# bacpop/ska.rust

Measured on AMD Instinct MI355X. Metric: genomes/sec ska build+align, 1 000x5 Mbp k=31; bit-exact vs CPU, higher is better.
Workload: dtype u64

## Files before the change

ska.rust_amd/csrc/skx_append.hip:

```cpp
#include "skx_device.h"
#include <cstdlib>
#include <type_traits>

namespace skx {

typedef uint32_t u32x4 __attribute__((ext_vector_type(4)));
typedef const u32x4 __attribute__((address_space(1))) *g4_t;

#ifdef SKX_AP_PROF
__device__ unsigned long long g_ap_prof[16];
#define AP_PROF_START unsigned long long tprof = __builtin_readcyclecounter(), tacc[12] = {0, 0, 0, 0, 0, 0, 0, 0, 0, 0, 0, 0}
#define AP_PROF(i) do { const unsigned long long t_ = __builtin_readcyclecounter(); tacc[(i)] += t_ - tprof; tprof = t_; } while (0)
#define AP_PROF_FLUSH() do { for (int i_ = 0; i_ < 12; i_++) if (tacc[i_] && (i_ >= 6 || (threadIdx.x & 63) == 0)) atomicAdd(&g_ap_prof[i_], tacc[i_]); } while (0)
extern "C" void skx_debug_phase_prof(unsigned long long *out, int reset)
{
    unsigned long long h[16];
    (void)hipDeviceSynchronize();
    (void)hipMemcpyFromSymbol(h, HIP_SYMBOL(g_ap_prof), sizeof(h));
    for (int i = 0; i < 16; i++) out[i] = h[i];
    if (reset) { for (auto &x : h) x = 0; (void)hipMemcpyToSymbol(HIP_SYMBOL(g_ap_prof), h, sizeof(h)); }
}
#else
#define AP_PROF_START do { } while (0)
#define AP_PROF(i) do { } while (0)
#define AP_PROF_FLUSH() do { } while (0)
#endif
#ifdef SKX_AP_PROF
#define AP_COUNT(i, v) do { tacc[(i)] += (v); } while (0)
#else
#define AP_COUNT(i, v) do { } while (0)
#endif

#ifndef AP_PRIO_L
#define AP_PRIO_L 1
#endif
#ifndef AP_PRIO_I
#define AP_PRIO_I 0
#endif
constexpr int AP_PRIO_STREAM = 3, AP_PRIO_LOOKUP = AP_PRIO_L, AP_PRIO_INSERT = AP_PRIO_I;
constexpr int AP_THREADS = 1024, AP_WAVES = 16;
constexpr uint32_t AP_PAD = 64;
constexpr uint32_t AP_Q = 256, AP_SQ = 64;
#ifndef AP_CH_N
#define AP_CH_N 8
#endif
#ifndef AP_RESYNC
#define AP_RESYNC 16
#endif
constexpr int AP_CH = AP_CH_N;
constexpr int AP_RANK_BITS = 14;
constexpr uint32_t AP_RANK_MASK = (1u << AP_RANK_BITS) - 1;

__device__ static inline uint32_t ap_wave_excl(uint32_t v, uint32_t *total)
{
    uint32_t inc = v;
#pragma unroll
    for (int d = 1; d < 64; d <<= 1) { const uint32_t t = __shfl_up(inc, d, 64); if ((int)(threadIdx.x & 63) >= d) inc += t; }
    *total = __shfl(inc, 63, 64);
    return inc - v;
}
__device__ static inline uint32_t ap_block_excl(uint32_t v, uint32_t *s_tmp , uint32_t *total)
{
    const int lane = threadIdx.x & 63, wv = threadIdx.x >> 6, nw = (blockDim.x + 63) >> 6;
    uint32_t wt;
    const uint32_t ex = ap_wave_excl(v, &wt);
    if (lane == 63) s_tmp[wv] = wt;
    __syncthreads();
    if (threadIdx.x == 0) { uint32_t run = 0; for (int i = 0; i < nw; i++) { const uint32_t t = s_tmp[i]; s_tmp[i] = run; run += t; } s_tmp[16] = run; }
    __syncthreads();
    const uint32_t r = s_tmp[wv] + ex;
    *total = s_tmp[16];
    __syncthreads();
    return r;
}
__device__ static inline uint32_t ap_mbcnt(unsigned long long b)
{
    return __builtin_amdgcn_mbcnt_hi((uint32_t)(b >> 32), __builtin_amdgcn_mbcnt_lo((uint32_t)b, 0u));
}

typedef volatile uint32_t __attribute__((address_space(3))) *lds_vol_t;
__device__ static inline lds_vol_t lds_vol(void *p) { return (lds_vol_t)(__attribute__((address_space(3))) void *)p; }
constexpr int CTL_NROWS = 0, CTL_FAIL = 1, CTL_TMP = 8, CTL_WORDS = 32;

static inline size_t append_lds_bytes(uint32_t nslots, uint32_t cap, bool count_only)
{
    size_t b = (size_t)(nslots + AP_PAD) * 8 + (size_t)(nslots + AP_PAD) + (size_t)AP_WAVES * (AP_Q + AP_SQ) * 8 + CTL_WORDS * 4;
    if (!count_only) b += (size_t)AP_WAVES * (cap / 8) * 4;
    return b;
}

template <bool COUNT_ONLY, bool HI>
__global__ __launch_bounds__(AP_THREADS) void append_kernel(AppendArgs a)
{
    extern __shared__ __attribute__((aligned(16))) unsigned char s_raw[];
    const uint32_t total_slots = a.nslots + AP_PAD;
    const uint32_t cap = a.cap, rbw = cap / 8;
    unsigned char *s_fp = s_raw;
    unsigned long long *s_tab = reinterpret_cast<unsigned long long *>(s_raw + total_slots);
    unsigned long long *s_q = s_tab + total_slots;
    uint32_t *s_ctl = reinterpret_cast<uint32_t *>(s_q + (size_t)AP_WAVES * (AP_Q + AP_SQ));
    uint32_t *s_rb = s_ctl + CTL_WORDS;
    const int tid = threadIdx.x, lane = tid & 63;
    const int wv = __builtin_amdgcn_readfirstlane(tid >> 6);
    const int S = a.n_samples;
    const int shA = a.logQ - a.logB;
    const uint32_t A = 1u << shA;
    const uint32_t G = gridDim.x;
    const bool xmap = a.logB >= 3 && G % (8u * A) == 0u;
    const int rem = a.bits - a.logQ;
    const int psh = rem + 4;
    const int lowb = HI ? rem - 32 : 0;
    const uint32_t fmask = HI ? (A - 1u) << (psh - 32) : 0u;
    uint32_t region = 0, part = 0, pshift = 0;
    uint64_t j = 0;
    uint8_t *piece0 = nullptr;
    unsigned long long *q = s_q + (size_t)wv * (AP_Q + AP_SQ), *sq = q + AP_Q;
    uint32_t *rb = s_rb + (size_t)wv * rbw;
    for (uint32_t rnd = 0; rnd < a.rounds; rnd++) {
    if (xmap) {
        const uint32_t xcd = blockIdx.x & 7u, ls = blockIdx.x >> 3, gpr = (G >> 3) >> shA;
        region = ((rnd * gpr + (ls >> shA)) << 3) + xcd; part = ls & (A - 1u);
    } else { const uint32_t blk = rnd * G + blockIdx.x; region = blk >> shA; part = blk & (A - 1u); }
    j = ((uint64_t)region << shA) + part;
    pshift = HI ? part << (psh - 32) : 0u;
    piece0 = a.pieces + j * (uint64_t)S * (cap / 2);

    for (uint32_t i = tid; i < total_slots; i += AP_THREADS) s_tab[i] = 0ull;
    for (uint32_t i = tid; i < total_slots / 4u; i += AP_THREADS) reinterpret_cast<uint32_t *>(s_fp)[i] = 0u;
    if (!COUNT_ONLY) for (uint32_t i = tid; i < AP_WAVES * rbw; i += AP_THREADS) s_rb[i] = 0u;
    if (tid < CTL_WORDS) s_ctl[tid] = 0u;
    if (tid == 0 && (uint32_t)(uintptr_t)(__attribute__((address_space(3))) unsigned char *)s_fp != 0u) atomicOr(a.overflow, 4);
    if (xmap && A > 1u && a.bar && tid == 0) {
        atomicAdd(&a.bar[region], 1);
        for (int it = 0; it < (1 << 18) && __hip_atomic_load(&a.bar[region], __ATOMIC_RELAXED, __HIP_MEMORY_SCOPE_AGENT) < (int)A; it++) __builtin_amdgcn_s_sleep(8);
    }
    __syncthreads();

    typedef const uint64_t __attribute__((address_space(4))) *cq_t;
    typedef const uint32_t __attribute__((address_space(4))) *c1_t;
    cq_t c_off = (cq_t)(uintptr_t)a.off;
    c1_t c_raw = (c1_t)(uintptr_t)a.raw;
    const uint64_t rstride = 1ull << a.logB;
    const uint32_t qbase = (uint32_t)(uintptr_t)(__attribute__((address_space(3))) unsigned long long *)q, qfull = qbase + 128u * 8u;
    uint32_t qw = qbase, nsq = 0;
    AP_PROF_START;
    __builtin_amdgcn_s_setprio(AP_PRIO_STREAM);

    auto key_hi = [&](uint32_t wlo, uint32_t whi) -> uint32_t {
        if (HI) return __builtin_amdgcn_alignbit(whi, wlo, (uint32_t)(rem - 28));
        return rem == 0 ? 0u : (uint32_t)(((wlo >> 4) | (whi << 28)) << (32 - rem));
    };
    const uint32_t hshift = (uint32_t)__builtin_clz(a.nslots) + 1u;
    auto home = [&](uint32_t kh) -> uint32_t { return kh >> hshift; };
    auto key_lo = [&](uint32_t wlo) -> uint32_t { return HI ? __builtin_amdgcn_ubfe(wlo, 4u, (uint32_t)lowb) << AP_RANK_BITS : 0u; };
    auto key_fp = [&](uint32_t kh, uint32_t kl) -> uint32_t {
        const uint32_t v = HI ? kh & 0xFFu : ((kh ^ (kl >> AP_RANK_BITS)) * 0x9E3779B1u) >> 24;
        return v | 1u;
    };
    auto record = [&](uint32_t rank1, uint32_t m4) {
        const uint32_t rank = rank1 - 1u;
        atomicOr(&rb[rank >> 3], m4 << ((rank & 7u) * 4u));
    };
    auto slow_batch = [&]() {
        __builtin_amdgcn_s_setprio(AP_PRIO_INSERT);
        const uint32_t take = nsq < 64u ? nsq : 64u;
        nsq -= take;
        if (lane == 0) { AP_COUNT(8, 1); AP_COUNT(9, take); }
        if ((uint32_t)lane < take) {
            const unsigned long long w = sq[nsq + lane];
            const uint32_t wlo = (uint32_t)w, whi = (uint32_t)(w >> 32);
            const uint32_t kh = key_hi(wlo, whi), kl = key_lo(wlo);
            const unsigned long long keyE = ((unsigned long long)kh << 32) | kl;
            uint32_t rank1 = 0;
            for (uint32_t t = home(kh); t + 3u < total_slots;) {
                AP_COUNT(10, 1); if (ap_mbcnt(__ballot(true)) == 0u) AP_COUNT(11, 1);
                const unsigned long long e0 = s_tab[t], e1 = s_tab[t + 1], e2 = s_tab[t + 2], e3 = s_tab[t + 3];
                const bool m0 = (e0 ^ keyE) - 1ull < AP_RANK_MASK, m1 = (e1 ^ keyE) - 1ull < AP_RANK_MASK, m2 = (e2 ^ keyE) - 1ull < AP_RANK_MASK, m3 = (e3 ^ keyE) - 1ull < AP_RANK_MASK;
                bool won = false;
                uint32_t at = 0;
                if (!(m0 | m1 | m2 | m3)) {
                    at = e0 == 0ull ? 0u : e1 == 0ull ? 1u : e2 == 0ull ? 2u : e3 == 0ull ? 3u : 4u;
                    if (at < 4u) won = atomicCAS(&s_tab[t + at], 0ull, keyE | AP_RANK_MASK) == 0ull;
                }
                if (won) {
                    const uint32_t mine = atomicAdd(&s_ctl[CTL_NROWS], 1u) + 1u;
                    if (mine > (COUNT_ONLY ? AP_RANK_MASK - 1u : cap)) s_ctl[CTL_FAIL] = 1u;
                    lds_vol(&s_tab[t + at])[0] = kl | (mine < AP_RANK_MASK ? mine : AP_RANK_MASK - 1u);
                    s_fp[t + at] = (unsigned char)key_fp(kh, kl);
                    rank1 = mine;
                }
                __builtin_amdgcn_wave_barrier();
                if (m0 | m1 | m2 | m3) {
                    const uint32_t mt = t + (m0 ? 0u : m1 ? 1u : m2 ? 2u : 3u);
                    uint32_t r = (uint32_t)(m0 ? e0 : m1 ? e1 : m2 ? e2 : e3) & AP_RANK_MASK;
                    for (int it = 0; it < (1 << 16) && r == AP_RANK_MASK; it++) r = lds_vol(&s_tab[mt])[0] & AP_RANK_MASK;
                    if (r == AP_RANK_MASK) { s_ctl[CTL_FAIL] = 1u; r = 0; }
                    rank1 = r;
                    break;
                }
                if (won) break;
                if (at == 4u) t += 4u;
            }
            if (rank1 > cap && !COUNT_ONLY) rank1 = 0;
            if (rank1 == 0) s_ctl[CTL_FAIL] = 1u;
            else if (!COUNT_ONLY) record(rank1, wlo & 15u);
        }
        __builtin_amdgcn_s_setprio(AP_PRIO_STREAM);
    };
    auto batch = [&](auto full_tag) {
        constexpr bool FULL = decltype(full_tag)::value;
        __builtin_amdgcn_s_setprio(AP_PRIO_LOOKUP);
        uint32_t nq = (qw - qbase) >> 3;
        const uint32_t take = FULL ? 128u : nq < 128u ? nq : 128u;
        nq -= take;
        qw -= take * 8u;
        if (lane == 0) { AP_COUNT(6, 1); AP_COUNT(7, take); }
        const bool va = FULL || (uint32_t)lane < take, vb = FULL || (uint32_t)lane + 64u < take;
        unsigned long long wa = 0, wb = 0;
        if (va) wa = q[nq + lane];
        if (vb) wb = q[nq + 64u + lane];
        const uint32_t alo = (uint32_t)wa, ahi = (uint32_t)(wa >> 32), blo = (uint32_t)wb, bhi = (uint32_t)(wb >> 32);
        const uint32_t kha = key_hi(alo, ahi), kla = key_lo(alo), khb = key_hi(blo, bhi), klb = key_lo(blo);
        const uint32_t hsa = home(kha), hsb = home(khb);
        auto where8 = [&](uint32_t hs, uint32_t fp) -> uint32_t {
            typedef const uint32_t __attribute__((address_space(3))) *lds_c32_t;
            const lds_c32_t f = (lds_c32_t)(uintptr_t)(hs & ~3u);
            const uint32_t fp4 = __builtin_amdgcn_perm(fp, fp, 0u);
            const uint32_t x0 = f[0] ^ fp4, x1 = f[1] ^ fp4;
            const uint32_t hs8 = hs << 3;
            const uint32_t z0 = (x0 - 0x01010101u) & ~x0 & (0x80808080u << (hs8 & 31u)), z1 = (x1 - 0x01010101u) & ~x1 & 0x80808080u;
            uint32_t p0, p1;
            asm("v_ffbl_b32 %0, %1" : "=v"(p0) : "v"(z0));
            asm("v_ffbl_b32 %0, %1" : "=v"(p1) : "v"(z1));
            p1 |= 32u;
            const uint32_t p = (p0 < p1 ? p0 : p1) & ~7u;
            return (hs8 & ~31u) + (p < 64u ? p : 64u);
        };
        const uint32_t oa = where8(hsa, key_fp(kha, kla)), ob = where8(hsb, key_fp(khb, klb));
        const unsigned long long ea = *reinterpret_cast<const unsigned long long *>(reinterpret_cast<const unsigned char *>(s_tab) + oa),
                                 eb = *reinterpret_cast<const unsigned long long *>(reinterpret_cast<const unsigned char *>(s_tab) + ob);
        const uint32_t ra0 = ((uint32_t)ea ^ kla) - 1u, rb0 = ((uint32_t)eb ^ klb) - 1u;
        const bool hita = va & ((uint32_t)(ea >> 32) == kha) & (ra0 < AP_RANK_MASK - 1u), hitb = vb & ((uint32_t)(eb >> 32) == khb) & (rb0 < AP_RANK_MASK - 1u);
        const unsigned long long xa = __builtin_amdgcn_ballot_w64(va & !hita), xb = __builtin_amdgcn_ballot_w64(vb & !hitb);
        if (!COUNT_ONLY) {
            if (hita) atomicOr(rb + __builtin_amdgcn_ubfe(ra0, 3u, 11u), (alo & 15u) << ((ra0 << 2) & 31u));
            if (hitb) atomicOr(rb + __builtin_amdgcn_ubfe(rb0, 3u, 11u), (blo & 15u) << ((rb0 << 2) & 31u));
        }
        if (xa | xb) {
            const uint32_t na = (uint32_t)__popcll(xa), nb = (uint32_t)__popcll(xb);
            if (nsq + na > AP_SQ) slow_batch();
            if (va & !hita) sq[nsq + ap_mbcnt(xa)] = wa;
            nsq += na;
            if (nsq + nb > AP_SQ) slow_batch();
            if (vb & !hitb) sq[nsq + ap_mbcnt(xb)] = wb;
            nsq += nb;
        }
        __builtin_amdgcn_s_setprio(AP_PRIO_STREAM);
    };

    u32x4 nxt[AP_CH];
    auto issue_one = [&](int r, uint64_t b) {
        const uint32_t vo = (uint32_t)lane * 16u;
        const uint64_t bq = b + (uint64_t)(r >> 2) * 4096u;
        switch (r & 3) {
        case 0: asm volatile("global_load_dwordx4 %0, %1, %2" : "=v"(nxt[r]) : "v"(vo), "s"(bq) : "memory"); break;
        case 1: asm volatile("global_load_dwordx4 %0, %1, %2 offset:1024" : "=v"(nxt[r]) : "v"(vo), "s"(bq) : "memory"); break;
        case 2: asm volatile("global_load_dwordx4 %0, %1, %2 offset:2048" : "=v"(nxt[r]) : "v"(vo), "s"(bq) : "memory"); break;
        default: asm volatile("global_load_dwordx4 %0, %1, %2 offset:3072" : "=v"(nxt[r]) : "v"(vo), "s"(bq) : "memory"); break;
        }
    };
    auto region_of = [&](int smp, uint64_t &off, uint32_t &cnt) { const uint64_t rr = (uint64_t)smp * rstride + region; off = c_off[rr]; cnt = c_raw[rr]; };
    if (wv < S) {
        int s = wv;
        uint64_t off_c, off_n = 0; uint32_t cnt_c, cnt_n = 0, c = 0;
        region_of(s, off_c, cnt_c);
        {
            const uint64_t b0 = (uint64_t)(uintptr_t)(a.words + off_c);
#pragma unroll
            for (int r = 0; r < AP_CH; r++) issue_one(r, b0);
        }
        for (;;) {
            AP_PROF(1);
            const uint32_t nch = (cnt_c + 64u * AP_CH * 2u - 1u) / (64u * AP_CH * 2u);
            const bool last_chunk = c + 1u >= nch;
            const bool more = !last_chunk || s + AP_WAVES < S;
            if (last_chunk && more) region_of(s + AP_WAVES, off_n, cnt_n);
            const uint64_t nb1 = (uint64_t)(uintptr_t)(a.words + (more && last_chunk ? off_n : off_c)) + (uint64_t)(more ? (last_chunk ? 0u : c + 1u) : c) * (64u * AP_CH * 16u);
            const uint32_t w0 = 2u * (c * (64u * AP_CH) + (uint32_t)lane);
            const uint32_t w0l = 2u * (uint32_t)lane, w1l = w0l + 1u;
            const int fill_left = (int)(cnt_c - c * (64u * AP_CH * 2u));
            const bool full_chunk = __builtin_amdgcn_readfirstlane((uint32_t)((c + 1u) * (64u * AP_CH * 2u) <= cnt_c)) != 0u;
#pragma unroll
            for (int r = 0; r < AP_CH; r++) {
                asm volatile("s_waitcnt vmcnt(%0)" :: "n"(AP_CH - 1) : "memory");
                AP_PROF(0);
                uint32_t alo, ahi, blo, bhi;
                if (HI) { alo = nxt[r].x; ahi = nxt[r].y; blo = nxt[r].z; bhi = nxt[r].w; }
                else {
                    asm volatile("v_mov_b32 %0, %1" : "=v"(alo) : "v"(nxt[r].x));
                    asm volatile("v_mov_b32 %0, %1" : "=v"(ahi) : "v"(nxt[r].y));
                    asm volatile("v_mov_b32 %0, %1" : "=v"(blo) : "v"(nxt[r].z));
                    asm volatile("v_mov_b32 %0, %1" : "=v"(bhi) : "v"(nxt[r].w));
                }
                const uint32_t widx = w0 + 128u * r;
#if defined(AP_X_NOFILTER)
                if (false) {
#else
                if (HI) {
#endif
                    unsigned long long ma, mb; uint32_t na, nb, ta, tb, qb, cA;
#define AP_FILTER_STEP(OFF) asm volatile("v_and_b32 %4, %9, %11\n\t" \
                                 "v_cmp_eq_u32_e64 %0, %10, %4\n\t" \
                                 "v_and_b32 %5, %9, %12\n\t" \
                                 "v_cmp_eq_u32_e64 %1, %10, %5\n\t" \
                                 "s_cmp_lg_u32 %16, 0\n\t" \
                                 "s_cbranch_scc1 .Lapf%=\n\t" \
                                 "s_sub_i32 %7, %13, " #OFF "\n\t" \
                                 "v_cmp_gt_i32_e32 vcc, %7, %14\n\t" \
                                 "s_and_b64 %0, %0, vcc\n\t" \
                                 "v_cmp_gt_i32_e32 vcc, %7, %15\n\t" \
                                 "s_and_b64 %1, %1, vcc\n" \
                                 ".Lapf%=:\n\t" \
                                 "s_bcnt1_i32_b64 %2, %0\n\t" \
                                 "s_bcnt1_i32_b64 %3, %1\n\t" \
                                 "s_lshl3_add_u32 %6, %2, %8\n\t" \
                                 "s_mov_b64 exec, %0\n\t" \
                                 "v_mbcnt_lo_u32_b32 %4, exec_lo, 0\n\t" \
                                 "v_mbcnt_hi_u32_b32 %4, exec_hi, %4\n\t" \
                                 "v_lshl_add_u32 %4, %4, 3, %8\n\t" \
                                 "ds_write2_b32 %4, %17, %11 offset1:1\n\t" \
                                 "s_mov_b64 exec, %1\n\t" \
                                 "v_mbcnt_lo_u32_b32 %5, exec_lo, 0\n\t" \
                                 "v_mbcnt_hi_u32_b32 %5, exec_hi, %5\n\t" \
                                 "v_lshl_add_u32 %5, %5, 3, %6\n\t" \
                                 "ds_write2_b32 %5, %18, %12 offset1:1\n\t" \
                                 "s_mov_b64 exec, -1\n\t" \
                                 "s_lshl3_add_u32 %8, %3, %6" \
                                 : "=&s"(ma), "=&s"(mb), "=&s"(na), "=&s"(nb), "=&v"(ta), "=&v"(tb), "=&s"(qb), "=&s"(cA), "+s"(qw) \
                                 : "s"(fmask), "s"(pshift), "v"(ahi), "v"(bhi), "s"(fill_left), "v"(w0l), "v"(w1l), "s"((uint32_t)full_chunk), "v"(alo), "v"(blo) \
                                 : "vcc", "scc", "memory")
                    static_assert(AP_CH <= 12, "one assembly text per load of a chunk");
                    switch (r) {
                    case 0: AP_FILTER_STEP(0); break; case 1: AP_FILTER_STEP(128); break; case 2: AP_FILTER_STEP(256); break; case 3: AP_FILTER_STEP(384); break;
                    case 4: AP_FILTER_STEP(512); break; case 5: AP_FILTER_STEP(640); break; case 6: AP_FILTER_STEP(768); break; case 7: AP_FILTER_STEP(896); break;
                    case 8: AP_FILTER_STEP(1024); break; case 9: AP_FILTER_STEP(1152); break; case 10: AP_FILTER_STEP(1280); break; default: AP_FILTER_STEP(1408); break;
                    }
#undef AP_FILTER_STEP
#if defined(AP_X_NOFILTER)
                } else if (alo == 0x12345u && bhi == 0x54321u) {
#else
                } else {
#endif
                    const uint32_t pa = (uint32_t)((((uint64_t)ahi << 32) | alo) >> psh), pb = (uint32_t)((((uint64_t)bhi << 32) | blo) >> psh);
                    const bool ka = widx < cnt_c && (pa & (A - 1u)) == part, kbb = widx + 1u < cnt_c && (pb & (A - 1u)) == part;
                    const unsigned long long ba = __ballot(ka), bb = __ballot(kbb);
                    const uint32_t na = (uint32_t)__popcll(ba), nb = (uint32_t)__popcll(bb);
                    const uint32_t nq = (qw - qbase) >> 3;
                    if (ka) q[nq + ap_mbcnt(ba)] = ((unsigned long long)ahi << 32) | alo;
                    if (kbb) q[nq + na + ap_mbcnt(bb)] = ((unsigned long long)bhi << 32) | blo;
                    qw += (na + nb) * 8u;
                }
                issue_one(r, nb1);
                AP_PROF(1);
#if defined(AP_X_NOBATCH)
                if (qw >= qfull) qw -= 128u * 8u;
#else
                while (qw >= qfull) { batch(std::true_type{}); AP_PROF(2);
#if defined(AP_X_NOSLOW)
                    if (nsq >= 64u) nsq -= 64u;
#else
                    while (nsq >= 64u) { slow_batch(); AP_PROF(3); }
#endif
                }
#endif
            }
            if (last_chunk) {
                while (qw != qbase) { batch(std::false_type{}); AP_PROF(2); while (nsq >= 64u) { slow_batch(); AP_PROF(3); } }
                while (nsq) { slow_batch(); AP_PROF(3); }
            }
            AP_PROF(1);
            if (last_chunk) {
                if (!COUNT_ONLY) {
                    uint32_t n = *lds_vol(&s_ctl[CTL_NROWS]);
                    n = __builtin_amdgcn_readfirstlane(n);
                    if (n > cap) n = cap;
                    uint8_t *dst = piece0 + (uint64_t)s * (cap / 2);
                    for (uint32_t v = lane; v * 32u < n; v += 64u) {
                        uint4 *src = reinterpret_cast<uint4 *>(rb) + v;
                        const uint4 x = *src;
                        *reinterpret_cast<uint4 *>(dst + v * 16u) = x;
                        *src = make_uint4(0u, 0u, 0u, 0u);
                    }
                    if (lane == 0) a.plen[j * (uint64_t)S + s] = (uint16_t)n;
                }
                AP_PROF(4);
                if (!more) break;
                s += AP_WAVES; c = 0; off_c = off_n; cnt_c = cnt_n;
                if (AP_RESYNC > 0) {
                    const int it = (s - wv) / AP_WAVES;
                    if (xmap && A > 1u && a.bar && it % (AP_RESYNC > 0 ? AP_RESYNC : 1) == 0 && it <= (S - AP_WAVES) / AP_WAVES) {
                        __syncthreads();
                        if (tid == 0) {
                            int *ctr = a.bar + (1 << a.logB) + region;
                            const int want = (int)A * (it / (AP_RESYNC > 0 ? AP_RESYNC : 1));
                            atomicAdd(ctr, 1);
                            for (int spin = 0; spin < (1 << 16) && __hip_atomic_load(ctr, __ATOMIC_RELAXED, __HIP_MEMORY_SCOPE_AGENT) < want; spin++) __builtin_amdgcn_s_sleep(4);
                        }
                        __syncthreads();
                    }
                }
            } else c++;
        }
        asm volatile("s_waitcnt vmcnt(0)" ::: "memory");
    }
    AP_PROF_FLUSH();
    __syncthreads();
    const uint32_t nr = s_ctl[CTL_NROWS];
    if (s_ctl[CTL_FAIL]) { if (tid == 0) atomicOr(a.overflow, (int)s_ctl[CTL_FAIL]); __syncthreads(); continue; }
    uint32_t *s_tmp = s_ctl + CTL_TMP;
    if (COUNT_ONLY) {
        uint32_t c = 0;
        for (uint32_t i = tid; i < total_slots; i += AP_THREADS) c += s_tab[i] != 0ull;
        uint32_t tot; (void)ap_block_excl(c, s_tmp, &tot);
        if (tid == 0) { atomicAdd(&a.probe[0], (unsigned long long)tot); atomicMax(&a.probe[1], (unsigned long long)tot); }
        continue;
    }
    uint16_t *s_perm = reinterpret_cast<uint16_t *>(s_q);
    for (uint32_t i = tid; i < cap; i += AP_THREADS) s_perm[i] = 0xFFFFu;
    __syncthreads();
    const uint32_t per = (total_slots + AP_THREADS - 1) / AP_THREADS;
    const uint32_t lo = tid * per, hi = lo + per < total_slots ? lo + per : total_slots;
    uint32_t c = 0;
    for (uint32_t i = lo; i < hi; i++) c += s_tab[i] != 0ull;
    uint32_t total;
    uint32_t pos = ap_block_excl(c, s_tmp, &total);
    uint64_t *slab = a.stage + j * (uint64_t)a.stride;
    for (uint32_t i = lo; i < hi; i++) {
        const unsigned long long e = s_tab[i];
        if (!e) continue;
        uint32_t gl = 0, lr = 0;
        for (int64_t t = (int64_t)i - 1; t >= 0; t--) { const unsigned long long o = s_tab[t]; if (!o) break; gl += o > e; }
        for (uint32_t t = i + 1; t < total_slots; t++) { const unsigned long long o = s_tab[t]; if (!o) break; lr += o < e; }
        const uint32_t idx = pos - gl + lr, rank = ((uint32_t)e & AP_RANK_MASK) - 1u;
        pos++;
        if (idx < a.stride && rank < cap) {
            uint64_t hl;
            if (HI) hl = ((uint64_t)(uint32_t)(e >> 32) << lowb) | (uint64_t)((uint32_t)e >> AP_RANK_BITS);
            else hl = rem == 0 ? 0ull : (uint64_t)((uint32_t)(e >> 32) >> (32 - rem));
            slab[idx] = ((((uint64_t)j << rem) | hl) << 4) | 1ull;
            s_perm[rank] = (uint16_t)idx;
        }
    }
    __syncthreads();
    uint16_t *pj = a.perm + j * (uint64_t)cap;
    for (uint32_t i = tid; i < cap; i += AP_THREADS) pj[i] = s_perm[i];
    if (tid == 0) { a.ncnt[j] = total; a.nrank[j] = nr < cap ? nr : cap; if (total > a.stride) atomicOr(a.overflow, 1); }
    __syncthreads();
    }
}

template <bool COUNT_ONLY>
static void launch_append_t(const AppendArgs &a, unsigned blocks, hipStream_t st)
{
    const size_t lds = append_lds_bytes(a.nslots, a.cap, COUNT_ONLY);
    const bool hi = a.bits - a.logQ >= 32;
    if (hi) {
        (void)hipFuncSetAttribute((const void *)append_kernel<COUNT_ONLY, true>, hipFuncAttributeMaxDynamicSharedMemorySize, (int)lds);
        hipLaunchKernelGGL((append_kernel<COUNT_ONLY, true>), dim3(blocks), dim3(AP_THREADS), lds, st, a);
    } else {
        (void)hipFuncSetAttribute((const void *)append_kernel<COUNT_ONLY, false>, hipFuncAttributeMaxDynamicSharedMemorySize, (int)lds);
        hipLaunchKernelGGL((append_kernel<COUNT_ONLY, false>), dim3(blocks), dim3(AP_THREADS), lds, st, a);
    }
}
bool append_ok(int bits, int logB, int logQ, uint32_t region_cap, uint32_t nslots, uint32_t cap)
{
    const int rem = bits - logQ;
    (void)region_cap;
    return logQ >= logB && rem >= 0 && rem <= 50 && cap % 128u == 0 && cap >= 128u && cap <= APPEND_MAX_CAP && nslots >= cap && (nslots & (nslots - 1u)) == 0u &&
           append_lds_bytes(nslots, cap, false) <= 160u * 1024u - 256u;
}
void launch_append(const AppendArgs &a, uint32_t region_cap, hipStream_t st) { (void)region_cap; launch_append_t<false>(a, (1u << a.logQ) / a.rounds, st); }
void launch_append_probe(const AppendArgs &a, uint32_t region_cap, unsigned blocks, hipStream_t st) { (void)region_cap; launch_append_t<true>(a, blocks, st); }

__device__ static inline uint32_t pieces_cut_block(const uint16_t *pl, int S, uint32_t cap, uint32_t min_count, uint32_t *s_hist)
{
    __shared__ uint32_t s_wave[4];
    __shared__ uint32_t s_cut;
    const uint32_t tid = threadIdx.x, lane = tid & 63u, wv = tid >> 6, nbin = cap + 1u, share = (nbin + 255u) / 256u;
    for (uint32_t i = tid; i < nbin; i += 256) s_hist[i] = 0;
    if (tid == 0) s_cut = 0;
    __syncthreads();
    for (int s = (int)tid; s < S; s += 256) { const uint32_t v = pl[s]; atomicAdd(&s_hist[v < cap ? v : cap], 1u); }
    __syncthreads();
    const uint32_t b0 = tid * share < nbin ? tid * share : nbin, b1 = b0 + share < nbin ? b0 + share : nbin;
    uint32_t own = 0;
    for (uint32_t b = b0; b < b1; b++) own += s_hist[b];
    uint32_t incl = own;
#pragma unroll
    for (int dd = 1; dd < 64; dd <<= 1) { const uint32_t o = (uint32_t)__shfl_down((int)incl, dd, 64); if (lane + (uint32_t)dd < 64u) incl += o; }
    if (lane == 0) s_wave[wv] = incl;
    __syncthreads();
    uint32_t above = incl - own;
    for (uint32_t w = wv + 1; w < 4; w++) above += s_wave[w];
    if (min_count >= 1u && above < min_count && min_count <= above + own) {
        uint32_t acc = above;
        for (uint32_t b = b1; b-- > b0;) { acc += s_hist[b]; if (acc >= min_count) { s_cut = b; break; } }
    }
    __syncthreads();
    const uint32_t rc = s_cut;
    __syncthreads();
    return rc;
}
__device__ static inline void pieces_cut_tally(uint32_t nr, uint32_t rc, unsigned long long *tally)
{
    const uint32_t lim = nr < rc ? nr : rc;
    const uint64_t seen = (uint64_t)((lim + 31u) / 32u) * 32u;
    if (seen < nr) { atomicAdd(&tally[0], (unsigned long long)(nr - seen)); atomicAdd(&tally[1], 1ull); }
}
__global__ __launch_bounds__(256) void pieces_cut_kernel(const uint16_t *plen, int S, uint32_t cap, uint32_t min_count, const uint32_t *nrank, const uint32_t *ncnt,
                                                         uint32_t stage, uint32_t *r_cut, unsigned long long *tally)
{
    extern __shared__ uint32_t s_hist[];
    const uint64_t j = blockIdx.x;
    const uint32_t cut = pieces_cut_block(plen + j * (uint64_t)S, S, cap, min_count, s_hist);
    if (threadIdx.x == 0) {
        uint32_t rc = min_count ? cut : 0xFFFFFFFFu;
        if (ncnt && ncnt[j] > stage) rc = 0xFFFFFFFFu;
        r_cut[j] = rc;
        if (tally && nrank) pieces_cut_tally(nrank[j], rc, tally);
    }
}
void launch_pieces_cut(const uint16_t *plen, int n_samples, uint32_t cap, uint32_t min_count, const uint32_t *nrank, const uint32_t *ncnt, uint32_t stage, int n_blocks,
                       uint32_t *r_cut, unsigned long long *tally, hipStream_t st)
{
    if (n_blocks <= 0) return;
    hipLaunchKernelGGL(pieces_cut_kernel, dim3((unsigned)n_blocks), dim3(256), ((size_t)cap + 1) * 4, st, plen, n_samples, cap, min_count, nrank, ncnt, stage, r_cut, tally);
}

__global__ __launch_bounds__(256) void pieces_stats_kernel(const uint8_t *pieces, const uint16_t *plen, const uint16_t *perm, const uint32_t *nrank, const uint32_t *ncnt,
                                                           const uint64_t *roff, uint32_t cap, int S, uint32_t *o_present, uint32_t *o_unambig, uint32_t *o_mask,
                                                           uint32_t *o_vcount, int force_direct, uint32_t stage, uint32_t min_count, unsigned long long *tally)
{
    constexpr int W = 4;
    extern __shared__ __attribute__((aligned(16))) uint16_t s_stage[];
    const uint32_t PS_STAGE = stage;
    uint16_t *const s_pr = s_stage, *const s_un = s_stage + stage, *const s_mk = s_stage + 2 * (size_t)stage;
    const uint64_t j = blockIdx.x;
    const uint32_t nr = nrank[j], nrows = ncnt[j];
    const uint64_t r0 = roff[j];
    if (blockIdx.y * 256u * 8u * W >= nr && !(blockIdx.y == 0 && nrows)) return;
    const bool staged = gridDim.y == 1 && nrows <= PS_STAGE && !force_direct;
    const int lane = threadIdx.x & 63, wv = __builtin_amdgcn_readfirstlane((int)(threadIdx.x >> 6));
    const uint16_t *pl = plen + j * (uint64_t)S;
    uint32_t lim = nr;
    if (min_count && staged) {
        const uint32_t rc = pieces_cut_block(pl, S, cap, min_count, reinterpret_cast<uint32_t *>(s_stage));
        if (threadIdx.x == 0 && tally) pieces_cut_tally(nr, rc, tally);
        if (rc < lim) lim = rc;
    }
    const uint32_t nseen = (lim + 31u) / 32u * 32u < nr ? (lim + 31u) / 32u * 32u : nr;
    const uint32_t ncol = (lim + 31u) / 32u, ncg = ncol < 64u ? ncol : 64u;
    uint32_t G = 4, P = 1;
    if (staged && ncol) {
        G = (ncol + 63u) / 64u;
        for (P = 4u / G; P > 1u && (P / 2u) * G * 36u * 4u * ncg > PS_STAGE * 6u; P >>= 1) { }
    }
    const uint32_t grp = (uint32_t)wv % G, slice = (uint32_t)wv / G;
    const uint32_t d = blockIdx.y * 256u + grp * 64u + (uint32_t)lane;
    const uint4 *col = reinterpret_cast<const uint4 *>(pieces + j * (uint64_t)S * (cap / 2)) + d;
    const uint32_t step = cap / 32;
    bool mine = slice < P && d * 32u < lim;
    const bool wave_has = slice < P && (d - (uint32_t)lane) * 32u < lim;
    uint32_t pN[W], aN[W];
    uint32_t pE[W], pO[W], aE[W], aO[W], uni[W];
    uint32_t PE0[W], PE1[W], PO0[W], PO1[W], AE0[W], AE1[W], AO0[W], AO1[W];
#pragma unroll
    for (int w = 0; w < W; w++) { pN[w] = aN[w] = 0; pE[w] = pO[w] = aE[w] = aO[w] = uni[w] = 0; PE0[w] = PE1[w] = PO0[w] = PO1[w] = AE0[w] = AE1[w] = AO0[w] = AO1[w] = 0; }
    auto nibfold = [&]() {
#pragma unroll
        for (int w = 0; w < W; w++) {
            pE[w] += pN[w] & 0x0F0F0F0Fu; pO[w] += (pN[w] >> 4) & 0x0F0F0F0Fu; aE[w] += aN[w] & 0x0F0F0F0Fu; aO[w] += (aN[w] >> 4) & 0x0F0F0F0Fu;
            pN[w] = aN[w] = 0;
        }
    };
    auto fold = [&]() {
        nibfold();
#pragma unroll
        for (int w = 0; w < W; w++) {
            PE0[w] += pE[w] & 0x00FF00FFu; PE1[w] += (pE[w] >> 8) & 0x00FF00FFu; PO0[w] += pO[w] & 0x00FF00FFu; PO1[w] += (pO[w] >> 8) & 0x00FF00FFu;
            AE0[w] += aE[w] & 0x00FF00FFu; AE1[w] += (aE[w] >> 8) & 0x00FF00FFu; AO0[w] += aO[w] & 0x00FF00FFu; AO1[w] += (aO[w] >> 8) & 0x00FF00FFu;
            pE[w] = pO[w] = aE[w] = aO[w] = 0;
        }
    };
    auto take = [&](int w, uint32_t x) {
        uint32_t t = x | (x >> 1); t |= t >> 2;
        const uint32_t nz = t & 0x11111111u;
        const uint32_t y = x & (x - nz);
        uint32_t u = y | (y >> 1); u |= u >> 2;
        const uint32_t am = u & 0x11111111u;
        pN[w] += nz; aN[w] += am;
        uni[w] |= x;
    };
    for (int s0 = (int)slice * 64, since = 0, nib = 0; wave_has && s0 < S; s0 += 64 * (int)P) {
        const uint32_t plv = s0 + lane < S ? (uint32_t)pl[s0 + lane] : 0u;
        const int n = S - s0 < 64 ? S - s0 : 64;
#pragma unroll 1
        for (int i0 = 0; i0 < n; i0 += 4) {
            if (nib == 12) { nibfold(); nib = 0; }
            nib += 4;
            uint4 x[4];
#pragma unroll
            for (int u = 0; u < 4; u++) {
                const uint32_t l = (uint32_t)__builtin_amdgcn_readlane((int)plv, (i0 + u) & 63);
                x[u] = make_uint4(0u, 0u, 0u, 0u);
                if (mine && i0 + u < n && d * 32u < l) x[u] = col[(uint64_t)(s0 + i0 + u) * step];
            }
#pragma unroll
            for (int u = 0; u < 4; u++) { take(0, x[u].x); take(1, x[u].y); take(2, x[u].z); take(3, x[u].w); }
        }
        since += 64;
        if (since >= 192) { fold(); since = 0; nib = 0; }
    }
    fold();
    if (P > 1u) {
        uint32_t *const xch = reinterpret_cast<uint32_t *>(s_stage);
        for (uint32_t half = P >> 1; half >= 1u; half >>= 1) {
            if (mine && slice >= half && slice < 2u * half) {
                uint32_t *const xa = xch + ((size_t)((slice - half) * G + grp) * 36u) * ncg + (uint32_t)lane;
#pragma unroll
                for (int w = 0; w < W; w++) {
                    uint32_t *q = xa + (size_t)w * 9u * ncg;
                    q[0] = PE0[w]; q[ncg] = PE1[w]; q[2 * ncg] = PO0[w]; q[3 * ncg] = PO1[w]; q[4 * ncg] = AE0[w]; q[5 * ncg] = AE1[w]; q[6 * ncg] = AO0[w]; q[7 * ncg] = AO1[w];
                    q[8 * ncg] = uni[w];
                }
            }
            __syncthreads();
            if (mine && slice < half) {
                const uint32_t *const xb = xch + ((size_t)(slice * G + grp) * 36u) * ncg + (uint32_t)lane;
#pragma unroll
                for (int w = 0; w < W; w++) {
                    const uint32_t *q = xb + (size_t)w * 9u * ncg;
                    PE0[w] += q[0]; PE1[w] += q[ncg]; PO0[w] += q[2 * ncg]; PO1[w] += q[3 * ncg]; AE0[w] += q[4 * ncg]; AE1[w] += q[5 * ncg]; AO0[w] += q[6 * ncg]; AO1[w] += q[7 * ncg];
                    uni[w] |= q[8 * ncg];
                }
            }
            __syncthreads();
        }
        if (slice) mine = false;
    }
    if (staged) {
        for (uint32_t p = threadIdx.x; p < nrows; p += 256) { s_pr[p] = 0; s_un[p] = 0; s_mk[p] = 0; }
        __syncthreads();
    }
    const uint16_t *pj = perm + j * (uint64_t)cap;
    if (mine) {
#pragma unroll
        for (int w = 0; w < W; w++) {
            uint32_t pres[8], amb[8];
            pres[0] = PE0[w] & 0xFFFFu; pres[4] = PE0[w] >> 16; pres[2] = PE1[w] & 0xFFFFu; pres[6] = PE1[w] >> 16;
            pres[1] = PO0[w] & 0xFFFFu; pres[5] = PO0[w] >> 16; pres[3] = PO1[w] & 0xFFFFu; pres[7] = PO1[w] >> 16;
            amb[0] = AE0[w] & 0xFFFFu; amb[4] = AE0[w] >> 16; amb[2] = AE1[w] & 0xFFFFu; amb[6] = AE1[w] >> 16;
            amb[1] = AO0[w] & 0xFFFFu; amb[5] = AO0[w] >> 16; amb[3] = AO1[w] & 0xFFFFu; amb[7] = AO1[w] >> 16;
            const uint4 pv = *reinterpret_cast<const uint4 *>(pj + d * 32u + (uint32_t)w * 8u);
            const uint32_t pw[4] = {pv.x, pv.y, pv.z, pv.w};
#pragma unroll
            for (int i = 0; i < 8; i++) {
                const uint32_t r = d * 32u + (uint32_t)w * 8u + i;
                if (r >= nr) break;
                const uint32_t p = (pw[i >> 1] >> (16 * (i & 1))) & 0xFFFFu;
                if (p >= nrows) continue;
                const uint32_t u = (uni[w] >> (4 * i)) & 15u;
                const uint32_t mk = ((u & 1u) << 1) | ((u & 2u) << 1) | ((u & 4u) << 2) | ((u & 8u) << 5);
                if (staged) { s_pr[p] = (uint16_t)pres[i]; s_un[p] = (uint16_t)(pres[i] - amb[i]); s_mk[p] = (uint16_t)mk; }
                else {
                    o_vcount[r0 + p] = pres[i];
                    __hip_atomic_store(&o_present[r0 + p], pres[i], __ATOMIC_RELAXED, __HIP_MEMORY_SCOPE_AGENT);
                    __hip_atomic_store(&o_unambig[r0 + p], pres[i] - amb[i], __ATOMIC_RELAXED, __HIP_MEMORY_SCOPE_AGENT);
                    o_mask[r0 + p] = mk;
                }
            }
        }
    }
    if (!staged) __threadfence();
    __syncthreads();
    const uint32_t rk0 = blockIdx.y * 256u * 8u * W, rk1 = rk0 + 256u * 8u * W < nseen ? rk0 + 256u * 8u * W : nseen;
    for (uint32_t rb = rk0 + (uint32_t)wv * 64u; rb < rk1; rb += 256u) {
        const uint32_t rr = rb + (uint32_t)lane;
        uint32_t pp = 0xFFFFu; bool hit = false;
        if (rr < rk1) {
            pp = pj[rr];
            if (pp < nrows) {
                if (staged) hit = s_un[pp] != s_pr[pp];
                else hit = __hip_atomic_load(&o_unambig[r0 + pp], __ATOMIC_RELAXED, __HIP_MEMORY_SCOPE_AGENT) != __hip_atomic_load(&o_present[r0 + pp], __ATOMIC_RELAXED, __HIP_MEMORY_SCOPE_AGENT);
            }
        }
        unsigned long long todo = __ballot(hit);
        while (todo) {
            const int src = __builtin_ctzll(todo);
            todo &= todo - 1;
            const uint32_t r = rb + (uint32_t)src, prow = (uint32_t)__shfl((int)pp, src, 64);
            uint32_t m = 0;
            for (int t = lane; t < S; t += 64) {
                if ((uint32_t)pl[t] <= r) continue;
                const uint32_t x = *(reinterpret_cast<const uint32_t *>(pieces + (j * (uint64_t)S + t) * (cap / 2)) + (r >> 3));
                const uint32_t nib = (x >> ((r & 7u) * 4u)) & 15u;
                if (nib) m |= 1u << nib;
            }
#pragma unroll
            for (int dd = 32; dd >= 1; dd >>= 1) m |= __shfl_xor(m, dd, 64);
            if (lane == 0) { if (staged) s_mk[prow] = (uint16_t)m; else o_mask[r0 + prow] = m; }
        }
    }
    if (!staged) return;
    __syncthreads();
    for (uint32_t p = threadIdx.x; p < nrows; p += 256) {
        const uint32_t pr = s_pr[p];
        o_present[r0 + p] = pr; o_vcount[r0 + p] = pr;
        o_unambig[r0 + p] = s_un[p]; o_mask[r0 + p] = s_mk[p];
    }
}
namespace {
struct StatsLaunch { unsigned gy; int direct; uint32_t stage; bool bounded() const { return gy == 1 && !direct; } };
StatsLaunch stats_launch(uint32_t cap)
{
    static const int direct = knob("stats_direct") ? 1 : 0;
    return {(cap / 32 + 255u) / 256u, direct, (cap + 63u) / 64u * 64u};
}
}
void launch_pieces_stats(const uint8_t *pieces, const uint16_t *plen, const uint16_t *perm, const uint32_t *nrank, const uint32_t *ncnt, const uint64_t *roff, uint32_t cap,
                         int n_samples, int n_blocks, uint32_t *present, uint32_t *unambig, uint32_t *mask, uint32_t *vcount, hipStream_t st, uint32_t min_count, unsigned long long *tally)
{
    if (n_blocks <= 0) return;
    const StatsLaunch l = stats_launch(cap);
    if (!l.bounded()) min_count = 0;
    hipLaunchKernelGGL(pieces_stats_kernel, dim3((unsigned)n_blocks, l.gy), dim3(256), (size_t)l.stage * 6, st, pieces, plen, perm, nrank, ncnt, roff, cap, n_samples, present, unambig, mask, vcount,
                       l.direct, l.stage, min_count, tally);
}
uint32_t pieces_stats_bound(uint32_t cap) { const StatsLaunch l = stats_launch(cap); return l.bounded() ? l.stage : 0u; }
__global__ __launch_bounds__(256) void pieces_cells_kernel(const uint8_t *pieces, const uint16_t *plen, uint32_t cap, int S, unsigned long long *out)
{
    const uint64_t j = blockIdx.x;
    const int lane = threadIdx.x & 63;
    for (int s = blockIdx.y * 4 + (threadIdx.x >> 6); s < S; s += gridDim.y * 4) {
        const uint32_t pl = plen[j * (uint64_t)S + s];
        const uint32_t *src = reinterpret_cast<const uint32_t *>(pieces + (j * (uint64_t)S + s) * (cap / 2));
        uint32_t c = 0;
        for (uint32_t i = lane; i < (pl + 7u) / 8u; i += 64) { const uint32_t x = src[i]; uint32_t t = x | (x >> 1); t |= t >> 2; c += (uint32_t)__popc(t & 0x11111111u); }
#pragma unroll
        for (int dd = 32; dd >= 1; dd >>= 1) c += __shfl_xor(c, dd, 64);
        if (lane == 0 && c) atomicAdd(&out[s], (unsigned long long)c);
    }
}
void launch_pieces_cells(const uint8_t *pieces, const uint16_t *plen, uint32_t cap, int n_samples, int n_blocks, unsigned long long *out, hipStream_t st)
{
    if (n_blocks <= 0 || n_samples <= 0) return;
    unsigned gy = (unsigned)((n_samples + 3) / 4); if (gy > 16) gy = 16;
    hipLaunchKernelGGL(pieces_cells_kernel, dim3((unsigned)n_blocks, gy), dim3(256), 0, st, pieces, plen, cap, n_samples, out);
}
__global__ __launch_bounds__(256) void region_totals_kernel(const uint32_t *raw, int logB, unsigned long long *out)
{
    __shared__ unsigned long long s_sum[256];
    const uint64_t B = 1ull << logB;
    unsigned long long t = 0;
    for (uint64_t b = threadIdx.x; b < B; b += 256) t += raw[(uint64_t)blockIdx.x * B + b];
    s_sum[threadIdx.x] = t;
    __syncthreads();
    for (int d = 128; d >= 1; d >>= 1) { if ((int)threadIdx.x < d) s_sum[threadIdx.x] += s_sum[threadIdx.x + d]; __syncthreads(); }
    if (threadIdx.x == 0) out[blockIdx.x] = s_sum[0];
}
void launch_region_totals(const uint32_t *raw, int n_samples, int logB, unsigned long long *out, hipStream_t st)
{
    if (n_samples > 0) hipLaunchKernelGGL(region_totals_kernel, dim3((unsigned)n_samples), dim3(256), 0, st, raw, logB, out);
}

constexpr int PR_WAVES = 8;
constexpr int PR_AHEAD = 3;
__device__ static inline uint32_t ap_iupac4(uint32_t m)
{
    const uint32_t idx = m & 0x07070707u;
    const uint32_t lo = __builtin_amdgcn_perm(0x48595754u, 0x4D43412Du, idx);
    const uint32_t hi = __builtin_amdgcn_perm(0x4E42444Bu, 0x56535247u, idx);
    const uint32_t sel = ((m >> 3) & 0x01010101u) * 0xFFu;
    return (hi & sel) | (lo & ~sel);
}
template <bool KEPT>
__global__ __launch_bounds__(64 * PR_WAVES) void pieces_rows_kernel(PiecesRowsArgs a)
{
    extern __shared__ __attribute__((aligned(16))) unsigned char s_raw[];
    const uint32_t cap = a.cap;
    uint16_t *s_src = reinterpret_cast<uint16_t *>(s_raw);
    uint32_t *s_piece = reinterpret_cast<uint32_t *>(s_raw + (((size_t)cap + 16) * 2 + 15) / 16 * 16);
    const uint64_t j = (uint64_t)blockIdx.x + a.j_base;
    const uint32_t n = a.ncnt[j];
    if (n == 0) return;
    const uint64_t r0 = a.roff[j];
    const uint64_t k0 = KEPT ? a.kpos[r0] : 0;
    const uint32_t nout = KEPT ? (uint32_t)(a.kpos[r0 + n] - k0) : n;
    if (nout == 0) return;
    const int tid = threadIdx.x, lane = tid & 63, wv = tid >> 6;
    const uint64_t ocol = KEPT ? k0 : r0 - a.col_base;
    const uint32_t shift = (uint32_t)(ocol & 3u);
    const uint32_t ndw = (nout + shift + 3u) / 4u;
    const uint16_t *pj = a.perm + j * (uint64_t)cap;
    const uint32_t nr = a.nrank[j];
    const int S = a.n_samples;
    const int s_lo = blockIdx.y * a.samples_per_wg, s_hi = s_lo + a.samples_per_wg < S ? s_lo + a.samples_per_wg : S;
    uint32_t *pc = s_piece + (size_t)wv * (cap / 8 + 4);
    const unsigned char *pcb = reinterpret_cast<const unsigned char *>(pc);
    __shared__ uint32_t s_top;
    uint32_t nrw = (nr + 7u) / 8u;
    if (lane < 4) pc[cap / 8 + lane] = 0u;
    for (uint32_t t0 = 0; t0 < nout + shift; t0 += cap) {
        for (uint32_t i = tid; i < cap + 16u; i += blockDim.x) s_src[i] = (uint16_t)cap;
        if (KEPT && tid == 0) s_top = 0;
        __syncthreads();
        uint32_t top = 0;
        for (uint32_t r = tid; r < nr; r += blockDim.x) {
            const uint32_t p = pj[r];
            if (p == 0xFFFFu || p >= n) continue;
            uint32_t sc;
            if (!KEPT) sc = shift + p;
            else if (a.keep[r0 + p] == 1) sc = shift + (uint32_t)(a.kpos[r0 + p] - k0);
            else continue;
            if (sc >= t0 && sc < t0 + cap) { s_src[sc - t0] = (uint16_t)r; top = r + 1u; }
        }
        if (KEPT && top) atomicMax(&s_top, top);
        __syncthreads();
        if (KEPT && !a.full_pieces) nrw = (s_top + 7u) / 8u;
        const uint32_t v_lo = t0 / 4u, v_hi = (t0 + cap) / 4u < ndw ? (t0 + cap) / 4u : ndw;
        const int cnt = __builtin_amdgcn_readfirstlane(s_lo + wv < s_hi ? (s_hi - s_lo - wv + PR_WAVES - 1) / PR_WAVES : 0);
        const uint32_t n4 = (nrw + 3u) / 4u;
        const uint16_t *plj = a.plen + j * (uint64_t)S + s_lo + wv;
        uint4 *pc4 = reinterpret_cast<uint4 *>(pc);
        auto masked = [&](uint4 x, uint32_t i, uint32_t plw) {
            if (4u * i >= plw) x.x = 0u;
            if (4u * i + 1u >= plw) x.y = 0u;
            if (4u * i + 2u >= plw) x.z = 0u;
            if (4u * i + 3u >= plw) x.w = 0u;
            return x;
        };
        uint32_t plv = 0, plw = 0, plw_next = 0;
        uint4 nx[PR_AHEAD];
#pragma unroll
        for (int u = 0; u < PR_AHEAD; u++) nx[u] = make_uint4(0u, 0u, 0u, 0u);
        auto ask = [&](int i) {
            if ((i & 63) == 0) plv = i + lane < cnt ? (uint32_t)plj[(size_t)(i + lane) * PR_WAVES] : 0u;
            plw_next = ((uint32_t)__builtin_amdgcn_readlane((int)plv, i & 63) + 7u) / 8u;
            const uint4 *src4 = reinterpret_cast<const uint4 *>(a.pieces + (j * (uint64_t)S + (uint64_t)(s_lo + wv + i * PR_WAVES)) * (cap / 2));
#pragma unroll
            for (int u = 0; u < PR_AHEAD; u++) { const uint32_t i4 = (uint32_t)lane + 64u * u; if (i4 < n4 && 4u * i4 < plw_next) nx[u] = src4[i4]; }
        };
        if (cnt > 0) ask(0);
        for (int it = 0; it < cnt; it++) {
            const int s = s_lo + wv + it * PR_WAVES;
            plw = plw_next;
#pragma unroll
            for (int u = 0; u < PR_AHEAD; u++) { const uint32_t i4 = (uint32_t)lane + 64u * u; if (i4 < n4) pc4[i4] = masked(nx[u], i4, plw); }
            if (n4 > 64u * PR_AHEAD) {
                const uint4 *src4 = reinterpret_cast<const uint4 *>(a.pieces + (j * (uint64_t)S + (uint64_t)s) * (cap / 2));
                for (uint32_t i4 = (uint32_t)lane + 64u * PR_AHEAD; i4 < n4; i4 += 64) pc4[i4] = masked(4u * i4 < plw ? src4[i4] : make_uint4(0u, 0u, 0u, 0u), i4, plw);
            }
            __builtin_amdgcn_wave_barrier();
            if (it + 1 < cnt) ask(it + 1);
            unsigned char *dst = a.out + (uint64_t)s * a.pitch + (ocol - shift);
            for (uint32_t v = v_lo + lane; v < v_hi; v += 64) {
                const uint2 rr = *reinterpret_cast<const uint2 *>(s_src + 4u * (v - v_lo));
                const uint32_t ra = rr.x & 0xFFFFu, rb = rr.x >> 16, rc = rr.y & 0xFFFFu, rd = rr.y >> 16;
                const uint32_t na = ((uint32_t)pcb[ra >> 1] >> ((ra & 1u) * 4u)) & 15u, nb = ((uint32_t)pcb[rb >> 1] >> ((rb & 1u) * 4u)) & 15u;
                const uint32_t nc = ((uint32_t)pcb[rc >> 1] >> ((rc & 1u) * 4u)) & 15u, nd = ((uint32_t)pcb[rd >> 1] >> ((rd & 1u) * 4u)) & 15u;
                uint32_t m = na | (nb << 8) | (nc << 16) | (nd << 24);
                uint32_t word = ap_iupac4(m);
                if (a.mask_ambig) {
                    const uint32_t y = m & (m - ((m | (m >> 1) | (m >> 2) | (m >> 3)) & 0x01010101u));
                    const uint32_t amb = ((y | (y >> 1) | (y >> 2) | (y >> 3)) & 0x01010101u) * 0xFFu;
                    word = (word & ~amb) | (0x4E4E4E4Eu & amb);
                }
                const bool head = v == 0 && shift != 0, tail = v == ndw - 1 && ((nout + shift) & 3u) != 0;
                if (!head && !tail) *reinterpret_cast<uint32_t *>(dst + 4u * v) = word;
                else {
#pragma unroll
                    for (int b = 0; b < 4; b++) { const int c = (int)(4u * v + b) - (int)shift; if (c >= 0 && (uint32_t)c < nout) dst[4u * v + b] = (unsigned char)(word >> (8 * b)); }
                }
            }
            __builtin_amdgcn_wave_barrier();
        }
        __syncthreads();
    }
}
void launch_pieces_rows(const PiecesRowsArgs &a, uint32_t n_blocks, hipStream_t st)
{
    if (!n_blocks || a.n_samples <= 0) return;
    PiecesRowsArgs b = a;
    int spw = a.n_samples;
    while (spw > PR_WAVES * 4 && (uint64_t)n_blocks * ((a.n_samples + spw - 1) / spw) < 8192) spw = (spw + 1) / 2;
    b.samples_per_wg = spw;
    const unsigned gy = (unsigned)((a.n_samples + spw - 1) / spw);
    const size_t lds = (((size_t)a.cap + 16) * 2 + 15) / 16 * 16 + (size_t)PR_WAVES * (a.cap / 8 + 4) * 4;
    if (a.keep) {
        (void)hipFuncSetAttribute((const void *)pieces_rows_kernel<true>, hipFuncAttributeMaxDynamicSharedMemorySize, (int)lds);
        hipLaunchKernelGGL(pieces_rows_kernel<true>, dim3(n_blocks, gy), dim3(64 * PR_WAVES), lds, st, b);
    } else {
        (void)hipFuncSetAttribute((const void *)pieces_rows_kernel<false>, hipFuncAttributeMaxDynamicSharedMemorySize, (int)lds);
        hipLaunchKernelGGL(pieces_rows_kernel<false>, dim3(n_blocks, gy), dim3(64 * PR_WAVES), lds, st, b);
    }
}

}

#include "skx_append_wide.inc"
```

ska.rust_amd/csrc/skx_device.h:

```cpp
#pragma once
#include <hip/hip_runtime.h>
#include <stdint.h>

namespace skx {

long knob(const char *name, long absent = 0);
int extract_tile_bases(int logB);
constexpr int MAX_LOGB = 13;
constexpr uint64_t EMPTY64 = ~0ull;

struct HashParams {
    int bits;
    int hb;
    uint32_t hmask;
    uint32_t c[4];
};
HashParams make_hash_params(int k);
__host__ __device__ inline uint32_t hround(uint32_t v, uint32_t c, int hb) { return (v * c) >> (32 - hb); }
__host__ __device__ inline void hmix_halves(uint32_t &L, uint32_t &R, const HashParams &p)
{
    L ^= hround(R, p.c[0], p.hb); R ^= hround(L, p.c[1], p.hb);
}
__host__ __device__ inline uint64_t hmix(uint64_t x, const HashParams &p)
{
    uint32_t L = (uint32_t)(x >> p.hb), R = (uint32_t)x & p.hmask;
    hmix_halves(L, R, p);
    return ((uint64_t)L << p.hb) | R;
}
__host__ __device__ inline uint64_t hunmix(uint64_t x, const HashParams &p)
{
    uint32_t L = (uint32_t)(x >> p.hb), R = (uint32_t)x & p.hmask;
    R ^= hround(L, p.c[1], p.hb); L ^= hround(R, p.c[0], p.hb);
    return ((uint64_t)L << p.hb) | R;
}

typedef unsigned __int128 u128;
struct WideHash { int bits, hb; uint64_t hmask; uint64_t c[3]; };
WideHash make_wide_hash(int k);
__host__ __device__ inline uint64_t hround64(uint64_t v, uint64_t c, int hb) { return (v * c) >> (64 - hb); }
__host__ __device__ inline void hmix_halves_w(uint64_t &L, uint64_t &R, const WideHash &p)
{
    L ^= hround64(R, p.c[0], p.hb); R ^= hround64(L, p.c[1], p.hb); L ^= hround64(R, p.c[2], p.hb);
}
__host__ __device__ inline u128 hunmix_w(u128 x, const WideHash &p)
{
    uint64_t L = (uint64_t)(x >> p.hb), R = (uint64_t)x & p.hmask;
    L ^= hround64(R, p.c[2], p.hb); R ^= hround64(L, p.c[1], p.hb); L ^= hround64(R, p.c[0], p.hb);
    return ((u128)L << p.hb) | R;
}
__host__ __device__ inline u128 hmix_w(u128 x, const WideHash &p)
{
    uint64_t L = (uint64_t)(x >> p.hb), R = (uint64_t)x & p.hmask;
    hmix_halves_w(L, R, p);
    return ((u128)L << p.hb) | R;
}

struct ExtractArgs {
    const uint8_t *const *seqs;
    const uint8_t *const *quals;
    const uint64_t *lens;
    int n_samples;
    int tiles_max;
    int parts = 0, tiles_part = 0;
    int k, rc;
    int min_qual, qual_filter;
    int logB;
    HashParams hp;
    WideHash wh;
    uint32_t *hist;
    const uint64_t *off;
    uint64_t *words;
    uint32_t capacity;
    int *overflow;
    uint32_t *sketch = nullptr;
};

constexpr int SKETCH_M = 18, SKETCH_COPIES = 8;
constexpr uint32_t SKETCH_WORDS = 1u << (SKETCH_M - 5);
constexpr double SKETCH_MAX_FILL = 0.5;
__host__ __device__ inline int sketch_step_log(int logB) { return logB >= 10 ? 8 : logB >= 8 ? 6 : 0; }
__host__ __device__ inline int sketch_regions(int logB) { return 1 << (logB - sketch_step_log(logB)); }
__host__ __device__ inline int sketch_shift64(int bits, int logB) { return (bits - logB < 32 ? bits - logB : 32) - SKETCH_M; }
__host__ __device__ inline uint32_t sketch_index64(uint32_t h, int shift) { return ((h * 0x9E3779B1u) >> shift) & ((1u << SKETCH_M) - 1u); }
inline bool sketch_ok(int bits, int logB) { return bits - logB >= SKETCH_M; }
inline size_t sketch_words(int logB) { return (size_t)SKETCH_COPIES * (size_t)sketch_regions(logB) * SKETCH_WORDS; }
void launch_sketch_count(const uint32_t *sketch, int logB, uint32_t *zeros, hipStream_t st);

void launch_hist(const ExtractArgs &a, hipStream_t st);
void launch_scatter(const ExtractArgs &a, hipStream_t st);

void launch_fill_offsets(uint64_t *off, uint64_t n, uint32_t capacity, hipStream_t st);
void launch_scan_u32(const uint32_t *in, uint64_t *out, uint64_t n, uint32_t *max_out, hipStream_t st);

constexpr int SUBIDX = 16;
uint32_t dedupe_spill_grid();
void launch_dedupe_mb(uint64_t *words, const uint64_t *off, const uint32_t *raw, uint32_t *ucnt, uint64_t n_regions,
                      uint32_t cap, int rem_bits, int *overflow, uint16_t *sidx, int sb, hipStream_t st,
                      uint32_t typical = 0, uint32_t *big_list = nullptr, uint32_t big_from = 0);

struct DictView {
    const uint64_t *words; const uint64_t *off; const uint32_t *ucnt;
    int n_samples, logB, bits;
    const uint16_t *sidx = nullptr; int sb = 0;
};

void launch_union(const DictView &d, int logN, uint64_t *stage, uint32_t stride, uint32_t *ncnt,
                  uint32_t table_slots, int *overflow, hipStream_t st);
void launch_union_probe(const DictView &d, int logP, int probe, uint32_t *cnt, uint32_t table_slots, int *overflow,
                        hipStream_t st);

struct AssembleArgs {
    DictView d;
    int logN;
    const uint64_t *stage;
    uint32_t stride;
    const uint32_t *ncnt;
    const uint64_t *roff;
    uint8_t *matrix;
    uint64_t pitch;
    uint32_t *col_present;
    uint32_t *col_unambig;
    uint32_t *col_mask;
    uint32_t max_rows;
    int *missing;
    uint32_t j_base = 0;
    uint64_t col_base = 0;
    const uint8_t *keep = nullptr; const uint64_t *kpos = nullptr;
    int mask_ambig = 0;
};
void launch_assemble(const AssembleArgs &a, hipStream_t st, int mode = 0, uint32_t n_blocks = 0);
bool union_side_ok(const DictView &d, int logN, uint32_t stride);
void launch_union_side(const DictView &d, int logN, uint64_t *stage, uint32_t stride, uint32_t *ncnt, uint32_t table_slots, int *overflow,
                       uint16_t *side, uint16_t *perm, hipStream_t st);
void launch_assemble_side(const AssembleArgs &a, const uint16_t *side, const uint16_t *perm, hipStream_t st, bool wide = false);
void launch_compose_perm(const uint64_t *l_stage, uint32_t l_stride, const uint32_t *l_ncnt, const uint16_t *l_perm, int l_logN, const uint64_t *g_stage,
                         uint32_t g_stride, const uint32_t *g_ncnt, const uint64_t *g_roff, int g_logN, int bits, uint16_t *g_perm, uint32_t *g_n,
                         uint64_t *g_base, uint32_t *g_max, int *bad, hipStream_t st);
void launch_union_side_wide(const DictView &d, int logN, u128 *stage, uint32_t stride, uint32_t *ncnt, uint32_t table_slots, int *overflow,
                            uint16_t *side, uint16_t *perm, hipStream_t st);

constexpr uint32_t APPEND_MAX_CAP = 6016, APPEND_MAX_SLOTS = 8192;
struct AppendArgs {
    const uint64_t *words; const uint64_t *off; const uint32_t *raw;
    int n_samples, logB, bits, logQ;
    uint32_t nslots, cap;
    uint8_t *pieces; uint16_t *plen; uint16_t *perm; uint32_t *nrank;
    uint64_t *stage; uint32_t stride; uint32_t *ncnt;
    unsigned long long *probe;
    int *overflow;
    uint32_t rounds = 1;
    int *bar = nullptr;
};
bool append_ok(int bits, int logB, int logQ, uint32_t region_cap, uint32_t nslots, uint32_t cap);
void launch_append(const AppendArgs &a, uint32_t region_cap, hipStream_t st);
void launch_append_probe(const AppendArgs &a, uint32_t region_cap, unsigned blocks, hipStream_t st);
constexpr uint32_t APPEND_WIDE_MAX_CAP = 3072, APPEND_WIDE_MAX_SLOTS = 4096;
bool append_wide_ok(int bits, int logB, int logQ, uint32_t nslots, uint32_t cap);
void launch_append_wide(const AppendArgs &a, hipStream_t st);
void launch_append_wide_probe(const AppendArgs &a, unsigned blocks, hipStream_t st);
void launch_pieces_stats(const uint8_t *pieces, const uint16_t *plen, const uint16_t *perm, const uint32_t *nrank, const uint32_t *ncnt, const uint64_t *roff, uint32_t cap,
                         int n_samples, int n_blocks, uint32_t *present, uint32_t *unambig, uint32_t *mask, uint32_t *vcount, hipStream_t st, uint32_t min_count = 0, unsigned long long *tally = nullptr);
void launch_pieces_cut(const uint16_t *plen, int n_samples, uint32_t cap, uint32_t min_count, const uint32_t *nrank, const uint32_t *ncnt, uint32_t stage, int n_blocks,
                       uint32_t *r_cut, unsigned long long *tally, hipStream_t st);
uint32_t pieces_stats_bound(uint32_t cap);
void launch_pieces_cells(const uint8_t *pieces, const uint16_t *plen, uint32_t cap, int n_samples, int n_blocks, unsigned long long *out, hipStream_t st);
void launch_region_totals(const uint32_t *raw, int n_samples, int logB, unsigned long long *out, hipStream_t st);
struct PiecesRowsArgs {
    const uint8_t *pieces; const uint16_t *plen; const uint16_t *perm; const uint32_t *nrank; uint32_t cap; int n_samples;
    const uint32_t *ncnt; const uint64_t *roff;
    uint8_t *out; uint64_t pitch;
    uint32_t j_base = 0; uint64_t col_base = 0;
    const uint8_t *keep = nullptr; const uint64_t *kpos = nullptr;
    int mask_ambig = 0;
    int full_pieces = 0;
    int samples_per_wg = 0;
};
void launch_pieces_rows(const PiecesRowsArgs &a, uint32_t n_blocks, hipStream_t st);

void launch_gather_keys(const uint64_t *stage, uint32_t stride, const uint32_t *ncnt, const uint64_t *roff, int n_sub,
                        uint64_t *out, int unhash, HashParams hp, hipStream_t st);
void launch_hash_keys(const uint64_t *keys, uint64_t *words, uint64_t n, HashParams hp, hipStream_t st);
void launch_keys_cbor(const uint64_t *words, uint64_t n, HashParams hp, uint8_t *out, int *short_key, hipStream_t st);
void launch_unhash_dict(const uint64_t *words, uint64_t n, uint64_t *keys, uint8_t *bases, HashParams hp, hipStream_t st);

void launch_col_stats(const uint8_t *matrix, uint64_t pitch, int n_samples, uint64_t n_cols, uint32_t *present,
                      uint32_t *unambig, uint32_t *mask, int *bad_byte, hipStream_t st);
struct FilterArgs {
    const uint32_t *vcount, *present, *unambig, *mask; uint64_t n_cols; uint32_t n_samples;
    uint64_t min_count; int ambig_as_missing, filter_type, ignore_const_gaps;
    uint8_t *keep;
    int two_stage = 0;
};
void launch_filter_flags(const FilterArgs &a, hipStream_t st);
void launch_row_stats_rm(const uint8_t *cells, uint64_t S, uint64_t nr, uint32_t *present, uint32_t *unambig, uint32_t *mask, int *bad_byte, hipStream_t st);
void launch_compact_rm(const uint8_t *cells, uint64_t S, uint64_t nr, const uint8_t *keep, const uint64_t *pos, uint8_t *out, uint64_t pitch,
                       uint64_t col0, int mask_ambig, hipStream_t st);
uint64_t scan_u8_blocks(uint64_t n);
void launch_scan_u8(const uint8_t *flags, uint64_t *pos, uint64_t n, uint32_t *sums, uint64_t *offs, hipStream_t st);
void launch_compact_matrix(const uint8_t *in, uint64_t in_pitch, uint8_t *out, uint64_t out_pitch, int n_samples,
                           uint64_t n_cols, const uint8_t *keep, const uint64_t *pos, int mask_ambig, hipStream_t st, const int *order = nullptr);
void launch_subset_verdicts(const uint8_t *matrix, uint64_t pitch, const int *order, int n, uint64_t n_cols, uint64_t min_count, int ambig_as_missing,
                            int filter_type, int ignore_const_gaps, uint8_t *keep, unsigned long long *counts, int *bad_byte, hipStream_t st);
void launch_compact_u32(const uint32_t *in, uint32_t *out, uint64_t n, const uint8_t *keep, const uint64_t *pos, hipStream_t st);
void launch_compact_stats(const uint32_t *const in[4], uint32_t *const out[4], uint64_t n, const uint8_t *keep, const uint64_t *pos, hipStream_t st);
void launch_compact_u64(const uint64_t *in, uint64_t *out, uint64_t n, const uint8_t *keep, const uint64_t *pos, hipStream_t st);
void launch_compact_u128(const uint64_t *in, uint64_t *out, uint64_t n, const uint8_t *keep, const uint64_t *pos, hipStream_t st);
void launch_mask_ambig_stats(uint32_t *mask, uint64_t n, hipStream_t st);
void launch_count_u8(const uint8_t *v, uint64_t n, uint8_t value, unsigned long long *out, hipStream_t st);
void launch_differ_u32(const uint32_t *a, const uint32_t *b, uint64_t n, int *flag, hipStream_t st);
void launch_transpose(const uint8_t *in, uint64_t in_pitch, uint64_t rows, uint64_t cols, uint8_t *out, uint64_t out_pitch,
                      hipStream_t st);
struct SnapChunk { uint64_t src_off, uoff; uint32_t src_len, ulen, crc, compressed; };
constexpr uint32_t SKF_SLOT = 8 + 65536;
int launch_skf_decode_cells(int device, const uint8_t *src, const SnapChunk *chunks, uint32_t n_chunks, uint64_t upos, uint64_t uend,
                            uint8_t *scratch , uint8_t *cells, uint64_t base_cell, int *status, hipStream_t st);
int launch_skf_encode_cells(int device, const uint8_t *cells, uint64_t base_cell, uint64_t upos, uint64_t uoff0, uint32_t n_chunks,
                            uint8_t *slots, uint32_t *sizes, hipStream_t st);
void launch_skf_gather(const uint8_t *slots, const uint32_t *sizes, const uint64_t *off, uint32_t n_chunks, uint8_t *dense, hipStream_t st);
void launch_row_nonmissing(const uint8_t *matrix, uint64_t pitch, int n_samples, uint64_t n_cols, unsigned long long *out,
                           hipStream_t st);

void launch_build_planes(const uint8_t *matrix, uint64_t pitch, int n_samples, uint64_t n_cols, uint64_t *planes, uint64_t wpr, int filt,
                         hipStream_t st, const int *order = nullptr);
void launch_keep_bits(const uint8_t *keep, const uint64_t *pos, uint64_t n, uint64_t *keep_bits, uint64_t *gpos, hipStream_t st);
void launch_split_keep(const uint8_t *keep, const uint32_t *col_mask, uint64_t n, uint8_t *clean, uint8_t *dirty, hipStream_t st, int mode = 0);
void launch_split_keep_from_dirty(uint8_t *dirty, uint64_t n, uint8_t *clean, hipStream_t st);
void launch_build_planes_keep(const uint8_t *matrix, uint64_t pitch, int n_samples, uint64_t n_cols, const uint64_t *keep_bits, const uint64_t *gpos,
                              uint64_t *planes, uint64_t wpr, int filt, hipStream_t st, uint32_t *first_group, uint64_t kept, const int *order = nullptr);
constexpr int DIST_NCOUNT = 16;
int launch_pair_counts(const uint64_t *planes, int n_samples, uint64_t words_per_row, int filt_ambig,
                       unsigned long long *out, hipStream_t st, int i_lo = 0, int i_hi = 0);

void launch_hist_wide(const ExtractArgs &a, hipStream_t st);
void launch_scatter_wide(const ExtractArgs &a, hipStream_t st);
int extract_tile_bases_wide();
void launch_dedupe_wide(u128 *words, const uint64_t *off, const uint32_t *raw, uint32_t *ucnt, uint64_t n_regions, uint32_t cap,
                        int rem_bits, int *overflow, uint16_t *sidx, int sb, hipStream_t st);
void launch_union_wide(const DictView &d, int logN, u128 *stage, uint32_t stride, uint32_t *ncnt, uint32_t table_slots, int *overflow,
                       hipStream_t st);
void launch_union_probe_wide(const DictView &d, int logP, int probe, uint32_t *cnt, uint32_t table_slots, int *overflow, hipStream_t st);
void launch_assemble_wide(const AssembleArgs &a, hipStream_t st, int mode = 0, uint32_t n_blocks = 0);
void launch_gather_keys_wide(const u128 *stage, uint32_t stride, const uint32_t *ncnt, const uint64_t *roff, int n_sub, u128 *out,
                             hipStream_t st);

uint64_t fasta_parse_tiles(uint64_t len);
#ifdef __HIPCC__
__device__ static inline void planes_bytes16(const uint64_t *groups, uint64_t t, uint64_t len, uint32_t sw[4], uint32_t qw[4])
{
    const uint64_t p0 = t * 16;
    const uint64_t *g = groups + (t >> 2) * 5;
    const int sh = (int)(t & 3) * 16;
    const uint32_t lo = (uint32_t)(g[0] >> sh) & 0xFFFFu, hi = (uint32_t)(g[1] >> sh) & 0xFFFFu, bad = (uint32_t)(g[2] >> sh) & 0xFFFFu,
                   nl = (uint32_t)(g[3] >> sh) & 0xFFFFu, qb = (uint32_t)(g[4] >> sh) & 0xFFFFu;
#pragma unroll
    for (int i = 0; i < 4; i++) {
        uint32_t x = 0, y = 0;
#pragma unroll
        for (int b = 0; b < 4; b++) {
            const int j = 4 * i + b;
            const uint32_t code = ((lo >> j) & 1u) | (((hi >> j) & 1u) << 1);
            const bool isnl = ((nl >> j) & 1u) || p0 + (uint64_t)j >= len;
            const uint32_t c = isnl ? 10u : ((bad >> j) & 1u) ? 78u : (0x47544341u >> (8 * code)) & 0xFFu;
            const uint32_t q = isnl ? 10u : ((qb >> j) & 1u) ? 33u : 32u;
            x |= c << (8 * b); y |= q << (8 * b);
        }
        sw[i] = x; qw[i] = y;
    }
}
#endif
void launch_expand_planes(const uint64_t *groups, uint64_t len, uint8_t *seq, uint8_t *qual, hipStream_t st);
void launch_fasta_parse(const uint8_t *const *raw, const uint64_t *rawlen, uint8_t *const *out, uint64_t *outlen, const uint32_t *tile_file,
                        const uint64_t *tile_base, uint64_t n_tiles, void *summary, uint64_t *tile_off, uint8_t *tile_kind, int n, hipStream_t st);

void launch_lookup_rows(const uint64_t *words, uint64_t n, const uint64_t *sorted, uint64_t m, uint32_t *idx, hipStream_t st);
void launch_lookup_rows_wide(const u128 *words, uint64_t n, const u128 *sorted, uint64_t m, uint32_t *idx, hipStream_t st);
void launch_hash_keys_wide(const u128 *keys, u128 *words, uint64_t n, const WideHash &wh, hipStream_t st);
void launch_map_lookup_wide(const uint64_t *wlo, const uint64_t *whi, const uint8_t *flag, const uint8_t *seq, uint64_t len, int h, const u128 *sorted,
                            const uint32_t *perm, uint64_t U, uint32_t *row, uint8_t *is_rc, hipStream_t st);
void launch_member_flags(const uint32_t *idx, uint64_t n, int reverse, uint8_t *keep, hipStream_t st);
void launch_scatter_rows(const uint8_t *src, uint64_t src_pitch, int n_samples, uint8_t *dst, uint64_t dst_pitch, const uint32_t *idx,
                         uint64_t n, hipStream_t st);
void launch_nonzero_flags(const uint32_t *v, uint64_t n, uint8_t *keep, hipStream_t st);

struct MapWriteArgs {
    const uint8_t *mv; uint64_t mpitch, M;
    const uint32_t *m_pos, *m_chrom;
    const uint64_t *mlo, *mhi;
    const uint8_t *refcat; uint64_t total;
    const uint64_t *clen, *coff; int n_chrom;
    uint64_t half; int ambig_mask;
    const uint64_t *repeat; uint64_t n_repeat;
    uint8_t *out; uint64_t opitch; int n_samples;
    uint32_t *pres; uint64_t ppitch;
    uint32_t *first, *last;
};
void launch_map_lookup(const uint64_t *wlo, const uint8_t *flag, const uint8_t *seq, uint64_t len, int h, const uint64_t *sorted,
                       const uint32_t *perm, uint64_t U, uint32_t *row, uint8_t *is_rc, hipStream_t st);
void launch_gather_mapped(const uint8_t *matrix, uint64_t pitch, int n_samples, const uint32_t *mapped, const uint32_t *row, const uint8_t *is_rc,
                          uint64_t M, uint8_t *mv, uint64_t mpitch, hipStream_t st);
void launch_aln_write(const MapWriteArgs &a, hipStream_t st);

}
```

ska.rust_amd/csrc/skx_merge.cpp:

```cpp
#include "skx_internal.h"
#include <algorithm>
#include <cmath>
#include <cstdlib>

using namespace skx;

extern "C" void skx_keyset_free(skx_keyset *ks) { delete ks; }
extern "C" int skx_keyset_size(const skx_keyset *ks, uint64_t *n) { *n = ks->total; return SKX_OK; }

static int keyset_finish(skx_keyset *ks)
{
    hipStream_t st = ks->ctx->stream;
    const uint64_t nsub = 1ull << ks->logN;
    SKX_TRY(ks->roff.alloc(nsub + 1));
    DevBuf<uint32_t> d_max; SKX_TRY(d_max.alloc(1));
    launch_scan_u32(ks->ncnt.p, ks->roff.p, nsub, d_max.p, st);
    SKX_HIP(hipMemcpyAsync(&ks->total, ks->roff.p + nsub, 8, hipMemcpyDeviceToHost, st));
    SKX_HIP(hipMemcpyAsync(&ks->max_rows, d_max.p, 4, hipMemcpyDeviceToHost, st));
    SKX_HIP(hipStreamSynchronize(st));
    if (getenv("SKX_DEBUG")) fprintf(stderr, "[skx] keyset: logN=%d sub-buckets=%llu rows=%llu mean=%.1f max=%u\n", ks->logN, (unsigned long long)nsub,
                                 (unsigned long long)ks->total, (double)ks->total / (double)nsub, ks->max_rows);
    return SKX_OK;
}

static void gather_row_keys(const skx_keyset *src, const uint32_t *ncnt, const uint64_t *roff, uint64_t *out, hipStream_t st)
{
    if (src->wide) launch_gather_keys_wide((const u128 *)src->stage.p, src->stride, ncnt, roff, 1 << src->logN, (u128 *)out, st);
    else launch_gather_keys(src->stage.p, src->stride, ncnt, roff, 1 << src->logN, out, 0, src->hp, st);
}

static int keyset_union_views(skx_ctx *ctx, const DictView &view, int k, int rc, HashParams hp, uint64_t est_hint, skx_keyset **out,
                              const skx_dictset *side_for = nullptr)
{
    const bool wide = k > 31;
    const WideHash wh = make_wide_hash(k);
    const int kbits = 2 * (k - 1);
    hipStream_t st = ctx->stream;
    DevBuf<int> d_flag; SKX_TRY(d_flag.alloc(1));
    const uint32_t table = wide ? 4096 : 8192, stride = wide ? 2048 : 4096, target = wide ? 1200 : 2500;
    int logN = std::max(std::max(0, view.logB), std::min(kbits, ilog2_ceil((est_hint + target - 1) / target)));
    DevBuf<uint16_t> side_buf;
    for (;; logN++) {
        std::unique_ptr<skx_keyset> ks(new skx_keyset());
        ks->ctx = ctx; ks->k = k; ks->rc = rc; ks->logN = logN; ks->hp = hp; ks->wh = wh; ks->wide = wide; ks->stride = stride;
        const uint64_t nsub = 1ull << logN;
        SKX_TRY(ks->stage.alloc(nsub * stride * ks->wpk())); SKX_TRY(ks->ncnt.alloc(nsub));
        SKX_TRY(d_flag.zero(st));
        const bool with_side = side_for && (wide || union_side_ok(view, logN, stride));
        if (wide && with_side) {
            if (!side_buf.p) SKX_TRY(side_buf.alloc(side_for->words.n / 2 + 64));
            SKX_TRY(ks->perm.alloc(nsub * stride));
            launch_union_side_wide(view, logN, (u128 *)ks->stage.p, stride, ks->ncnt.p, table, d_flag.p, side_buf.p, ks->perm.p, st);
            ks->side_of = side_for;
        } else if (wide) launch_union_wide(view, logN, (u128 *)ks->stage.p, stride, ks->ncnt.p, table, d_flag.p, st);
        else if (with_side) {
            if (!side_buf.p) SKX_TRY(side_buf.alloc(side_for->words.n));
            SKX_TRY(ks->perm.alloc(nsub * stride));
            launch_union_side(view, logN, ks->stage.p, stride, ks->ncnt.p, 7168u, d_flag.p, side_buf.p, ks->perm.p, st);
            ks->side_of = side_for;
        } else launch_union(view, logN, ks->stage.p, stride, ks->ncnt.p, table, d_flag.p, st);
        int overflow = 0;
        SKX_HIP(hipMemcpyAsync(&overflow, d_flag.p, 4, hipMemcpyDeviceToHost, st));
        SKX_HIP(hipStreamSynchronize(st));
        SKX_HIP(hipGetLastError());
        if (overflow) {
            if (logN >= kbits) { set_error("key union overflow"); return SKX_EUNSUP; }
            continue;
        }
        SKX_TRY(keyset_finish(ks.get()));
        if (ks->side_of) ks->side = std::move(side_buf);
        *out = ks.release();
        return SKX_OK;
    }
}

struct TablesView { DevBuf<uint64_t> off; DevBuf<uint32_t> ucnt; DictView v; };
static int tables_view(TablesView &tv, const uint64_t *words, const uint64_t *h_off, const uint32_t *h_cnt, int n, int k, hipStream_t st)
{
    SKX_TRY(tv.off.alloc(n + 1)); SKX_TRY(tv.ucnt.alloc(n));
    SKX_HIP(hipMemcpyAsync(tv.off.p, h_off, (size_t)(n + 1) * 8, hipMemcpyHostToDevice, st));
    SKX_HIP(hipMemcpyAsync(tv.ucnt.p, h_cnt, (size_t)n * 4, hipMemcpyHostToDevice, st));
    tv.v = DictView{words, tv.off.p, tv.ucnt.p, n, 0, 2 * (k - 1)};
    return SKX_OK;
}

int skx::keyset_union_tables(skx_ctx *ctx, const uint64_t *words, const std::vector<uint64_t> &h_off, const std::vector<uint32_t> &h_cnt, int k, int rc,
                             skx_keyset **out)
{
    hipStream_t st = ctx->stream;
    const int n_sets = (int)h_cnt.size();
    StageTimer t(ctx, &ctx->tm.key_union);
    uint64_t total = 0, maxn = 0;
    for (int i = 0; i < n_sets; i++) { total += h_cnt[i]; maxn = std::max<uint64_t>(maxn, h_cnt[i]); }
    TablesView tv; SKX_TRY(tables_view(tv, words, h_off.data(), h_cnt.data(), n_sets, k, st));
    int r = keyset_union_views(ctx, tv.v, k, rc, make_hash_params(std::min(k, 31)), std::min(total, maxn * 2), out);
    SKX_HIP(hipStreamSynchronize(st));
    return r;
}

int skx::keyset_flatten(skx_keyset *ks)
{
    if (ks->flat.p) return SKX_OK;
    SKX_TRY(ks->flat.alloc(ks->total * ks->wpk()));
    gather_row_keys(ks, ks->ncnt.p, ks->roff.p, ks->flat.p, ks->ctx->stream);
    return SKX_OK;
}

extern "C" int skx_keyset_device(skx_keyset *ks, const void **dptr, uint64_t *n_keys, int *words_per_key)
{
    return skx_guarded([&]() -> int {
    SKX_HIP(hipSetDevice(ks->ctx->device));
    SKX_TRY(keyset_flatten(ks));
    SKX_HIP(hipStreamSynchronize(ks->ctx->stream));
    *dptr = ks->flat.p; *n_keys = ks->total; if (words_per_key) *words_per_key = ks->wpk();
    return SKX_OK;
    });
}

extern "C" int skx_keyset_from_device(skx_ctx *ctx, const void *dptr, uint64_t n_keys, int k, int rc, skx_keyset **out)
{
    return skx_guarded([&]() -> int {
    SKX_TRY(check_k(k));
    SKX_HIP(hipSetDevice(ctx->device));
    std::unique_ptr<skx_keyset> ks(new skx_keyset());
    ks->ctx = ctx; ks->k = k; ks->rc = rc; ks->hp = make_hash_params(std::min(k, 31)); ks->wh = make_wide_hash(k); ks->wide = k > 31; ks->logN = -1; ks->total = n_keys;
    SKX_TRY(ks->flat.alloc(n_keys * ks->wpk()));
    SKX_HIP(hipMemcpyAsync(ks->flat.p, dptr, n_keys * 8 * ks->wpk(), hipMemcpyDeviceToDevice, ctx->stream));
    SKX_HIP(hipStreamSynchronize(ctx->stream));
    *out = ks.release();
    return SKX_OK;
    });
}

extern "C" int skx_keyset_merge(skx_ctx *ctx, skx_keyset *const *sets, int n_sets, skx_keyset **out)
{
    return skx_guarded([&]() -> int {
    if (!ctx || !sets || n_sets <= 0 || !out) { set_error("bad arguments"); return SKX_EINVAL; }
    SKX_HIP(hipSetDevice(ctx->device));
    hipStream_t st = ctx->stream;
    uint64_t total = 0;
    for (int i = 0; i < n_sets; i++) {
        if (sets[i]->k != sets[0]->k) { set_error("K-mer lengths do not match: %d %d", sets[i]->k, sets[0]->k); return SKX_EINVAL; }
        if (sets[i]->rc != sets[0]->rc) { set_error("Strand use inconsistent"); return SKX_EINVAL; }
        if (sets[i]->logN >= 0) SKX_TRY(keyset_flatten(sets[i]));
        total += sets[i]->total;
    }
    DevBuf<uint64_t> words;
    const int wpk = sets[0]->wpk();
    SKX_TRY(words.alloc(total * wpk));
    std::vector<uint64_t> h_off(n_sets + 1, 0); std::vector<uint32_t> h_cnt(n_sets);
    for (int i = 0; i < n_sets; i++) {
        if (sets[i]->total > 0xFFFFFFFFull) { set_error("keyset too large"); return SKX_EUNSUP; }
        h_cnt[i] = (uint32_t)sets[i]->total; h_off[i + 1] = h_off[i] + sets[i]->total;
        SKX_HIP(hipMemcpyAsync(words.p + h_off[i] * wpk, sets[i]->flat.p, sets[i]->total * 8 * wpk, hipMemcpyDeviceToDevice, st));
    }
    return keyset_union_tables(ctx, words.p, h_off, h_cnt, sets[0]->k, sets[0]->rc, out);
    });
}

extern "C" void skx_array_free(skx_array *a) { delete a; }
extern "C" const char *skx_array_name(const skx_array *a, uint64_t i) { return i < a->names.size() ? a->names[i].c_str() : ""; }
extern "C" const char *skx_array_version(const skx_array *a) { return a->version.c_str(); }
extern "C" int skx_array_info(const skx_array *a, skx_array_info_t *info)
{
    return skx_guarded([&]() -> int {
    info->k = a->k; info->rc = a->rc; info->k_bits = a->k_bits; info->n_kmers = a->n_kmers; info->n_rows = a->n_rows;
    info->n_samples = a->names.size();
    info->total_samples = a->total_samples ? a->total_samples : a->names.size();
    return SKX_OK;
    });
}

static int new_array(skx_ctx *ctx, const skx_dictset *d, const char *const *names, uint64_t U, std::unique_ptr<skx_array> &a)
{
    a.reset(new skx_array());
    a->ctx = ctx; a->k = d->k; a->rc = d->rc; a->k_bits = d->key_bits; a->hp = d->hp; a->wh = d->wh; a->version = skx_version();
    for (int i = 0; i < d->n; i++) a->names.emplace_back(names && names[i] ? names[i] : "");
    a->n_rows = a->n_kmers = U; a->pitch = 0; a->engine_order = true;
    SKX_TRY(a->present.alloc(U)); SKX_TRY(a->unambig.alloc(U)); SKX_TRY(a->mask.alloc(U)); SKX_TRY(a->keys.alloc(U * (d->wide() ? 2 : 1))); SKX_TRY(a->vcount.alloc(U));
    return SKX_OK;
}

static AssembleArgs assemble_args(const skx_dictset *d, const skx_keyset *rows, skx_array *a, int *d_flag)
{
    AssembleArgs aa{};
    aa.d = d->view(); aa.logN = rows->logN; aa.stage = rows->stage.p; aa.stride = rows->stride; aa.ncnt = rows->ncnt.p; aa.roff = rows->roff.p;
    aa.matrix = nullptr; aa.pitch = 0; aa.col_present = a->present.p; aa.col_unambig = a->unambig.p; aa.col_mask = a->mask.p;
    aa.max_rows = rows->max_rows; aa.missing = d_flag;
    return aa;
}
static int check_missing(skx_ctx *ctx, const int *d_flag)
{
    int missing = 0;
    SKX_HIP(hipMemcpyAsync(&missing, d_flag, 4, hipMemcpyDeviceToHost, ctx->stream));
    SKX_HIP(hipStreamSynchronize(ctx->stream));
    SKX_HIP(hipGetLastError());
    if (missing) { set_error("row keyset does not contain every split k-mer of the samples"); return SKX_EINVAL; }
    return SKX_OK;
}

int skx::pieces_stats_pass(skx_array *a, uint64_t min_count, DevBuf<unsigned long long> *tally)
{
    skx_ctx *ctx = a->ctx; hipStream_t st = ctx->stream;
    const skx_pieces *pc = a->pieces; const skx_keyset *blk = a->lazy_rows;
    const int S = (int)a->names.size(), nb = 1 << pc->logQ;
    if (!a->n_rows) return SKX_OK;
    const bool bounded = min_count >= 2 && tally && pieces_stats_bound(pc->cap);
    if (bounded) { SKX_TRY(tally->alloc(2)); SKX_TRY(tally->zero(st)); }
    {
        StageTimer t(ctx, &ctx->tm.assemble);
        KernelTimer kt(ctx, &ctx->tm.pieces_stats);
        launch_pieces_stats(pc->data.p, pc->plen.p, pc->perm.p, pc->nrank.p, blk->ncnt.p, blk->roff.p, pc->cap, S, nb, a->present.p, a->unambig.p, a->mask.p, a->vcount.p, st,
                            bounded ? (uint32_t)std::min<uint64_t>(min_count, 0xFFFFFFFEull) : 0u, bounded ? tally->p : nullptr);
    }
    if (!bounded) SKX_HIP(hipStreamSynchronize(st));
    SKX_HIP(hipGetLastError());
    return SKX_OK;
}

static int append_not_taken(skx_ctx *ctx, const char *why)
{
    ctx->merge_path = std::string("sorted: ") + why;
    if (getenv("SKX_DEBUG")) fprintf(stderr, "[skx] merge: %s\n", ctx->merge_path.c_str());
    return SKF_NOT_TAKEN;
}
static bool append_fits(bool wide, int bits, int logB, int lq, uint32_t region_cap, uint32_t nslots, uint32_t cap) { return wide ? append_wide_ok(bits, logB, lq, nslots, cap) : append_ok(bits, logB, lq, region_cap, nslots, cap); }
static uint32_t append_max_cap(bool wide) { return wide ? APPEND_WIDE_MAX_CAP : APPEND_MAX_CAP; }
static uint32_t append_max_slots(bool wide) { return wide ? APPEND_WIDE_MAX_SLOTS : APPEND_MAX_SLOTS; }
static double ranks_need(double mean, double est_relvar) { return mean + 6.0 * std::sqrt(mean + 1.0 + est_relvar * mean * mean) + 32.0; }
static uint32_t ranks_for(double mean, double est_relvar, uint32_t max_cap)
{
    return (uint32_t)std::min<double>(max_cap, std::ceil(ranks_need(mean, est_relvar) / 128.0) * 128.0);
}
static uint32_t slots_for(uint32_t cap, uint32_t max_slots)
{
    uint32_t n = 256u;
    while (n < cap + cap / 3 && n < max_slots) n <<= 1;
    return n;
}

struct RowEstimate { double u_est = 0, est_relvar = 0; char sized[160] = "one sample"; };
static int estimate_rows(skx_ctx *ctx, const skx_dictset *d, AppendArgs aa, int min_logQ, uint64_t raw_max, RowEstimate &e)
{
    hipStream_t st = ctx->stream;
    const bool wide = d->wide();
    const int logB = d->logB, bits = aa.bits;
    e.u_est = (double)raw_max;
    if (d->n <= 1) return SKX_OK;
    if (d->sketch.p && !knob("probe_launch")) {
        const int nsk = sketch_regions(logB);
        DevBuf<uint32_t> d_zeros; SKX_TRY(d_zeros.alloc(nsk));
        { KernelTimer kt(ctx, &ctx->tm.append_probe); launch_sketch_count(d->sketch.p, logB, d_zeros.p, st); }
        std::vector<uint32_t> zeros(nsk);
        SKX_HIP(hipMemcpyAsync(zeros.data(), d_zeros.p, (size_t)nsk * 4, hipMemcpyDeviceToHost, st));
        SKX_HIP(hipStreamSynchronize(st));
        SKX_HIP(hipGetLastError());
        const double M = (double)(1u << SKETCH_M);
        double rows = 0, var = 0, fill = 0;
        for (uint32_t z : zeros) {
            fill = std::max(fill, 1.0 - (double)z / M);
            if (z == 0) continue;
            const double t = -std::log((double)z / M);
            rows += M * t; var += M * (std::exp(t) - t - 1.0);
        }
        if (fill <= SKETCH_MAX_FILL) {
            const double scale = (double)(1u << sketch_step_log(logB));
            e.u_est = std::max((double)raw_max * 0.5, rows * scale);
            e.est_relvar = rows > 0 ? var / (rows * rows) : 0.0;
            snprintf(e.sized, sizeof e.sized, "the sketch: %.1f rows in %d sketch regions, fill %.3f", rows, nsk, fill);
            return SKX_OK;
        }
        snprintf(e.sized, sizeof e.sized, "the probe launch: the sketch is %.3f full", fill);
    } else snprintf(e.sized, sizeof e.sized, "the probe launch: %s", d->sketch.p ? "SKX_KNOBS=probe_launch" : "no sketch");
    const double target = wide ? 2600.0 : 5400.0;
    DevBuf<unsigned long long> d_probe; SKX_TRY(d_probe.alloc(2));
    aa.probe = d_probe.p;
    int logP = std::min(bits, std::max(min_logQ, ilog2_ceil((uint64_t)((double)raw_max * 3.0 / target) + 1)));
    for (int attempt = 0;; attempt++) {
        const unsigned blocks = (unsigned)std::min<uint64_t>(64, 1ull << logP);
        aa.logQ = logP; aa.nslots = append_max_slots(wide); aa.cap = append_max_cap(wide); aa.rounds = 1; aa.bar = nullptr;
        if (!append_fits(wide, bits, logB, logP, d->region_cap, aa.nslots, aa.cap))
            return append_not_taken(ctx, "no probe split with room for a rank in a table entry (very short or very long hash)");
        SKX_HIP(hipMemsetAsync(aa.overflow, 0, sizeof(int), st)); SKX_TRY(d_probe.zero(st));
        { KernelTimer kt(ctx, &ctx->tm.append_probe); if (wide) launch_append_wide_probe(aa, blocks, st); else launch_append_probe(aa, d->region_cap, blocks, st); }
        unsigned long long pr[2] = {0, 0}; int ov = 0;
        SKX_HIP(hipMemcpyAsync(pr, d_probe.p, 16, hipMemcpyDeviceToHost, st));
        SKX_HIP(hipMemcpyAsync(&ov, aa.overflow, 4, hipMemcpyDeviceToHost, st));
        SKX_HIP(hipStreamSynchronize(st));
        SKX_HIP(hipGetLastError());
        if (!ov) { e.u_est = std::max((double)raw_max * 0.5, (double)pr[0] / blocks * (double)(1ull << logP)); return SKX_OK; }
        if (ov & 4) return append_not_taken(ctx, "the table's bytes are not at LDS address 0");
        if (attempt >= 4 || logP + 2 > bits) return append_not_taken(ctx, "the probe blocks kept overflowing");
        logP += 2;
    }
}

struct AppendSplit { uint32_t cap, nslots; uint64_t amp; bool allowed; uint32_t rounds; uint64_t grid; };
static AppendSplit append_split(double u_est, double est_relvar, int logQ, int logB, uint32_t region_cap, bool wide, int cus, uint64_t raw_sum)
{
    AppendSplit s{};
    const uint64_t nsub = 1ull << logQ;
    s.cap = ranks_for(u_est / (double)nsub, est_relvar, append_max_cap(wide)); s.nslots = slots_for(s.cap, append_max_slots(wide));
    s.amp = 1ull << (logQ - logB);
    const uint64_t amp_max = region_cap > lds_sort_max(wide) ? 32 : 8;
    s.allowed = !(s.amp > amp_max && (double)raw_sum * (double)s.amp > 4e8);
    uint64_t g = nsub;
    while (g > (uint64_t)std::max(cus, 1) && g % 2 == 0) g /= 2;
    const bool persistent = g <= (uint64_t)std::max(cus, 1) && nsub % g == 0 && g % (8 * s.amp) == 0 && logB >= 3;
    s.grid = persistent ? g : 0; s.rounds = persistent ? (uint32_t)(nsub / g) : 1;
    return s;
}

static int append_pass(skx_ctx *ctx, skx_dictset *d, std::unique_ptr<skx_keyset> &ks_out, std::unique_ptr<skx_pieces> &pc_out)
{
    if (d->sorted) return append_not_taken(ctx, "the dictionaries are sorted (read sets, oversize or repeat-rich samples, SKX_KNOBS=sorted_dicts)");
    if (d->n > 65535 || d->n < 1) return append_not_taken(ctx, "more than 65535 samples");
    SKX_HIP(hipSetDevice(ctx->device));
    hipStream_t st = ctx->stream;
    const bool wide = d->wide();
    const int S = d->n, bits = wide ? d->wh.bits : d->hp.bits, logB = d->logB, wpk = wide ? 2 : 1;
    uint64_t raw_sum = 0, raw_max = 0;
    for (auto v : d->raw_total) { raw_sum += v; raw_max = std::max(raw_max, v); }
    const int min_logQ = std::max(logB, bits - (wide ? 113 : 50));
    if (min_logQ > bits) return append_not_taken(ctx, "no row-block split with room for a rank in a table entry");
    DevBuf<int> d_flag; SKX_TRY(d_flag.alloc(1));
    AppendArgs aa{};
    aa.words = d->words.p; aa.off = d->off.p; aa.raw = d->raw.p; aa.n_samples = S; aa.logB = logB; aa.bits = bits; aa.overflow = d_flag.p;
    StageTimer t(ctx, &ctx->tm.key_union);
    RowEstimate e;
    SKX_TRY(estimate_rows(ctx, d, aa, min_logQ, raw_max, e));
    int logQ = min_logQ;
    while (logQ < bits && ranks_need(e.u_est / (double)(1ull << logQ), e.est_relvar) > (double)append_max_cap(wide)) logQ++;
    if (knob("append_coarse") > 0) logQ = std::max<long>(min_logQ, logQ - knob("append_coarse"));
    int cus = 0; (void)hipDeviceGetAttribute(&cus, hipDeviceAttributeMultiprocessorCount, ctx->device);
    for (int attempt = 0;; attempt++, logQ++) {
        if (logQ > bits || attempt > 3) return append_not_taken(ctx, "row blocks kept overflowing (a sample that is one repeat, or far more rows than the probe saw)");
        const uint64_t nsub = 1ull << logQ;
        const AppendSplit sp = append_split(e.u_est, e.est_relvar, logQ, logB, d->region_cap, wide, cus, raw_sum);
        if (!sp.allowed) return append_not_taken(ctx, "too many row blocks per region: every region would be read too often");
        if (!append_fits(wide, bits, logB, logQ, d->region_cap, sp.nslots, sp.cap)) return append_not_taken(ctx, "no row-block split that fits the LDS");
        std::unique_ptr<skx_keyset> ks(new skx_keyset());
        ks->ctx = ctx; ks->k = d->k; ks->rc = d->rc; ks->logN = logQ; ks->hp = d->hp; ks->wh = d->wh; ks->wide = wide; ks->stride = sp.cap;
        std::unique_ptr<skx_pieces> pc(new skx_pieces());
        pc->cap = sp.cap; pc->logQ = logQ;
        SKX_TRY(ks->stage.alloc(nsub * sp.cap * wpk)); SKX_TRY(ks->ncnt.alloc(nsub));
        if (pc->data.alloc(nsub * (uint64_t)S * (sp.cap / 2)) != SKX_OK) return append_not_taken(ctx, "no room for the pieces");
        SKX_TRY(pc->plen.alloc(nsub * (uint64_t)S + 2)); SKX_TRY(pc->perm.alloc(nsub * sp.cap)); SKX_TRY(pc->nrank.alloc(nsub));
        SKX_TRY(d_flag.zero(st));
        DevBuf<int> d_bar;
        if (sp.grid) { SKX_TRY(d_bar.alloc(2ull << logB)); SKX_TRY(d_bar.zero(st)); }
        aa.logQ = logQ; aa.nslots = sp.nslots; aa.cap = sp.cap; aa.rounds = sp.rounds; aa.bar = d_bar.p;
        aa.pieces = pc->data.p; aa.plen = pc->plen.p; aa.perm = pc->perm.p; aa.nrank = pc->nrank.p;
        aa.stage = ks->stage.p; aa.stride = sp.cap; aa.ncnt = ks->ncnt.p;
        { KernelTimer kt(ctx, &ctx->tm.append); if (wide) launch_append_wide(aa, st); else launch_append(aa, d->region_cap, st); }
        int ov = 0;
        SKX_HIP(hipMemcpyAsync(&ov, d_flag.p, 4, hipMemcpyDeviceToHost, st));
        SKX_HIP(hipStreamSynchronize(st));
        SKX_HIP(hipGetLastError());
        if (getenv("SKX_DEBUG")) fprintf(stderr, "[skx] append%s: logQ=%d (x%llu per region) cap=%u slots=%u rows~%.0f -> %s [sized by %s]\n", wide ? " (128-bit keys)" : "", logQ, (unsigned long long)sp.amp, sp.cap, sp.nslots, e.u_est, ov ? "overflow" : "ok", e.sized);
        if (ov & 4) return append_not_taken(ctx, "the table's bytes are not at LDS address 0");
        if (ov) continue;
        SKX_TRY(keyset_finish(ks.get()));
        ctx->merge_path = wide ? "append128" : "append64";
        ks_out = std::move(ks); pc_out = std::move(pc);
        return SKX_OK;
    }
}

static int array_over_pieces(skx_ctx *ctx, const skx_dictset *d, skx_keyset *ks, skx_pieces *pc_, skx_keyset *g, const char *const *names, skx_array **out)
{
    std::unique_ptr<skx_pieces> pc(pc_);
    hipStream_t st = ctx->stream;
    const int logQ = pc->logQ;
    const uint64_t nsub = 1ull << logQ;
    std::unique_ptr<skx_keyset> blk(new skx_keyset());
    blk->ctx = ctx; blk->k = d->k; blk->rc = d->rc; blk->logN = logQ; blk->hp = d->hp; blk->wh = d->wh; blk->wide = d->wide(); blk->stride = pc->cap;
    uint64_t U;
    if (g) {
        U = g->total;
        pc->perm = std::move(g->g_perm);
        blk->ncnt = std::move(g->g_n);
        SKX_TRY(blk->roff.alloc(nsub + 1));
        SKX_HIP(hipMemcpyAsync(blk->roff.p, g->g_base.p, nsub * 8, hipMemcpyDeviceToDevice, st));
        SKX_HIP(hipMemcpyAsync(blk->roff.p + nsub, &U, 8, hipMemcpyHostToDevice, st));
        SKX_HIP(hipStreamSynchronize(st));
        g->g_base.release();
        blk->total = U; blk->max_rows = g->g_max;
    } else {
        U = ks->total;
        SKX_TRY(blk->ncnt.alloc(nsub)); SKX_TRY(blk->roff.alloc(nsub + 1));
        SKX_HIP(hipMemcpyAsync(blk->ncnt.p, ks->ncnt.p, nsub * 4, hipMemcpyDeviceToDevice, st));
        SKX_HIP(hipMemcpyAsync(blk->roff.p, ks->roff.p, (nsub + 1) * 8, hipMemcpyDeviceToDevice, st));
        blk->total = U; blk->max_rows = ks->max_rows;
    }
    std::unique_ptr<skx_array> a;
    SKX_TRY(new_array(ctx, d, names, U, a));
    if (U) {
        if (g) gather_row_keys(g, g->ncnt.p, g->roff.p, a->keys.p, st);
        else gather_row_keys(ks, blk->ncnt.p, blk->roff.p, a->keys.p, st);
        if (g) { SKX_TRY(a->present.zero(st)); SKX_TRY(a->unambig.zero(st)); SKX_TRY(a->mask.zero(st)); SKX_TRY(a->vcount.zero(st)); }
    }
    a->pieces = pc.release(); a->lazy_rows = blk.release();
    a->stats_ready = g || knob("stats_eager");
    if (a->stats_ready) SKX_TRY(pieces_stats_pass(a.get(), 0));
    SKX_HIP(hipStreamSynchronize(st));
    SKX_HIP(hipGetLastError());
    *out = a.release();
    return SKX_OK;
}
static int merge_append(skx_ctx *ctx, skx_dictset *d, const char *const *names, skx_array **out)
{
    std::unique_ptr<skx_keyset> ks; std::unique_ptr<skx_pieces> pc;
    const int r = append_pass(ctx, d, ks, pc);
    if (r != SKX_OK) return r;
    return array_over_pieces(ctx, d, ks.get(), pc.release(), nullptr, names, out);
}

static int keyset_union_dict(skx_ctx *ctx, skx_dictset *d, skx_keyset **out, bool with_side)
{
    if (!ctx || !d || !out) { set_error("bad arguments"); return SKX_EINVAL; }
    SKX_HIP(hipSetDevice(ctx->device));
    hipStream_t st = ctx->stream;
    if (with_side && !d->sorted && !d->wide()) {
        std::unique_ptr<skx_keyset> ks; std::unique_ptr<skx_pieces> pc;
        const int r = append_pass(ctx, d, ks, pc);
        if (r == SKX_OK) { ks->pieces = pc.release(); ks->pieces_of = d; ks->pieces_of_id = d->id; *out = ks.release(); return SKX_OK; }
        if (r != SKF_NOT_TAKEN) return r;
    }
    if (!d->sorted && d->wide() && with_side) ctx->merge_path = "sorted: the key-table exchange of a sharded job composes 64-bit rows only";
    else if (!d->sorted && !with_side) ctx->merge_path = "sorted: a row set without cells was asked for (skx_keyset_union)";
    SKX_TRY(dictset_sort(d));
    StageTimer t(ctx, &ctx->tm.key_union);
    DictView v = d->view();
    uint64_t maxs = 0, sum = 0;
    for (auto s : d->sample_size) { maxs = std::max(maxs, s); sum += s; }
    uint64_t est = maxs;
    if (d->n > 1) {
        const int logP = std::min(2 * (d->k - 1), std::max(d->logB, ilog2_ceil((sum + 1023) / 1024)));
        const int probe = (int)std::min<uint64_t>(64, 1ull << logP);
        DevBuf<uint32_t> d_cnt; DevBuf<int> d_flag;
        SKX_TRY(d_cnt.alloc(1)); SKX_TRY(d_flag.alloc(1)); SKX_TRY(d_cnt.zero(st)); SKX_TRY(d_flag.zero(st));
        if (d->wide()) launch_union_probe_wide(v, logP, probe, d_cnt.p, 4096, d_flag.p, st);
        else launch_union_probe(v, logP, probe, d_cnt.p, 8192, d_flag.p, st);
        uint32_t cnt = 0; int ov = 0;
        SKX_HIP(hipMemcpyAsync(&cnt, d_cnt.p, 4, hipMemcpyDeviceToHost, st));
        SKX_HIP(hipMemcpyAsync(&ov, d_flag.p, 4, hipMemcpyDeviceToHost, st));
        SKX_HIP(hipStreamSynchronize(st));
        if (!ov) est = std::max<uint64_t>(maxs, (uint64_t)((double)cnt * (double)(1ull << logP) / probe * 1.1));
        else est = sum;
    }
    return keyset_union_views(ctx, v, d->k, d->rc, d->hp, est, out, with_side ? d : nullptr);
}
extern "C" int skx_keyset_union(skx_ctx *ctx, skx_dictset *d, skx_keyset **out)
{
    return skx_guarded([&]() -> int { return keyset_union_dict(ctx, d, out, false); });
}
extern "C" int skx_keyset_union_notes(skx_ctx *ctx, skx_dictset *d, skx_keyset **out)
{
    return skx_guarded([&]() -> int { return keyset_union_dict(ctx, d, out, true); });
}

extern "C" int skx_array_assemble(skx_ctx *ctx, skx_dictset *d, skx_keyset *rows, const char *const *names, skx_array **out)
{
    return skx_guarded([&]() -> int {
    if (!ctx || !d || !rows || !out) { set_error("bad arguments"); return SKX_EINVAL; }
    if (rows->k != d->k) { set_error("K-mer lengths do not match: %d %d", d->k, rows->k); return SKX_EINVAL; }
    if (rows->rc != d->rc) { set_error("Strand use inconsistent"); return SKX_EINVAL; }
    if (d->n > 65535) { set_error("more than 65535 samples per device array"); return SKX_EUNSUP; }
    SKX_HIP(hipSetDevice(ctx->device));
    hipStream_t st = ctx->stream;
    if (rows->holds_pieces_of(d)) {
        skx_pieces *pc = rows->pieces; rows->pieces = nullptr; rows->pieces_of = nullptr;
        return array_over_pieces(ctx, d, rows, pc, rows->g_perm.p ? rows : nullptr, names, out);
    }
    SKX_TRY(dictset_sort(d));
    std::unique_ptr<skx_keyset> rebuilt;
    if (rows->logN < 0 || rows->logN < d->logB) {
        if (rows->logN >= 0) SKX_TRY(keyset_flatten(rows));
        const uint64_t h_off[2] = {0, rows->total}; const uint32_t h_cnt = (uint32_t)rows->total;
        TablesView tv; SKX_TRY(tables_view(tv, rows->flat.p, h_off, &h_cnt, 1, rows->k, st));
        skx_keyset *tmp = nullptr;
        uint64_t hint = std::max<uint64_t>(rows->total, (uint64_t)2500 << d->logB);
        SKX_TRY(keyset_union_views(ctx, tv.v, rows->k, rows->rc, rows->hp, hint, &tmp));
        SKX_HIP(hipStreamSynchronize(st));
        rebuilt.reset(tmp);
        rows = tmp;
        if (rows->logN < d->logB) { set_error("internal: keyset granularity"); return SKX_EUNSUP; }
    }
    const uint64_t U = rows->total;
    std::unique_ptr<skx_array> a;
    SKX_TRY(new_array(ctx, d, names, U, a));
    a->pitch = pitch_for(U);
    SKX_TRY(a->matrix.alloc((uint64_t)d->n * a->pitch));
    DevBuf<int> d_flag; SKX_TRY(d_flag.alloc(1)); SKX_TRY(d_flag.zero(st));
    if (U) {
        AssembleArgs aa = assemble_args(d, rows, a.get(), d_flag.p);
        aa.matrix = a->matrix.p; aa.pitch = a->pitch;
        {
            StageTimer t(ctx, &ctx->tm.assemble);
            if (rows->g_perm.p && rows->side.p && rows->side_of == d && !rebuilt && !rows->wide) {
                AssembleArgs ag = aa;
                ag.logN = rows->l_logN; ag.stride = rows->l_stride; ag.ncnt = rows->g_n.p; ag.roff = rows->g_base.p; ag.max_rows = rows->g_max;
                launch_assemble_side(ag, rows->side.p, rows->g_perm.p, st, false);
            }
            else if (rows->side.p && !rows->g_perm.p && rows->side_of == d && !rebuilt) launch_assemble_side(aa, rows->side.p, rows->perm.p, st, rows->wide);
            else if (rows->wide) launch_assemble_wide(aa, st);
            else launch_assemble(aa, st);
        }
        gather_row_keys(rows, rows->ncnt.p, rows->roff.p, a->keys.p, st);
        SKX_HIP(hipMemcpyAsync(a->vcount.p, a->present.p, U * 4, hipMemcpyDeviceToDevice, st));
    }
    SKX_TRY(check_missing(ctx, d_flag.p));
    *out = a.release();
    return SKX_OK;
    });
}

static int array_make_lazy(skx_ctx *ctx, skx_dictset *d, skx_keyset *rows, const char *const *names, skx_array **out)
{
    std::unique_ptr<skx_dictset> own_d(d); std::unique_ptr<skx_keyset> own_rows(rows);
    rows->side.release(); rows->perm.release(); rows->g_perm.release(); rows->g_n.release(); rows->g_base.release(); rows->side_of = nullptr;
    std::unique_ptr<skx_array> a;
    SKX_TRY(new_array(ctx, d, names, rows->total, a));
    a->lazy_dict = own_d.release(); a->lazy_rows = own_rows.release(); a->stats_ready = false;
    if (a->n_rows) gather_row_keys(rows, rows->ncnt.p, rows->roff.p, a->keys.p, ctx->stream);
    SKX_HIP(hipStreamSynchronize(ctx->stream));
    *out = a.release();
    return SKX_OK;
}
extern "C" int skx_array_assemble_lazy(skx_ctx *ctx, skx_dictset *d, skx_keyset *rows, const char *const *names, skx_array **out)
{
    return skx_guarded([&]() -> int {
    if (!ctx || !d || !rows || !out) { skx_dictset_free(d); skx_keyset_free(rows); set_error("bad arguments"); return SKX_EINVAL; }
    if (rows->holds_pieces_of(d) || rows->wide != d->wide() || rows->k != d->k || rows->rc != d->rc || rows->logN < 0 || rows->logN < d->logB || d->n > 65535 ||
        knob("eager_array")) {
        const int r = skx_array_assemble(ctx, d, rows, names, out);
        skx_dictset_free(d); skx_keyset_free(rows);
        return r;
    }
    SKX_HIP(hipSetDevice(ctx->device));
    { const int rs = dictset_sort(d); if (rs != SKX_OK) { skx_dictset_free(d); skx_keyset_free(rows); return rs; } }
    return array_make_lazy(ctx, d, rows, names, out);
    });
}

static void launch_assemble_lazy(skx_array *a, const AssembleArgs &aa, hipStream_t st, int mode, uint32_t n_blocks = 0)
{
    if (a->lazy_rows->wide) launch_assemble_wide(aa, st, mode, n_blocks); else launch_assemble(aa, st, mode, n_blocks);
}
int skx::array_lazy_stats(skx_array *a)
{
    if (!a->lazy() || a->stats_ready) return SKX_OK;
    skx_ctx *ctx = a->ctx; hipStream_t st = ctx->stream;
    SKX_HIP(hipSetDevice(ctx->device));
    if (a->pieces) {
        ctx->cut_ranks = ctx->cut_blocks = 0;
        SKX_TRY(pieces_stats_pass(a, 0));
        a->stats_ready = true;
        return SKX_OK;
    }
    DevBuf<int> d_flag; SKX_TRY(d_flag.alloc(1)); SKX_TRY(d_flag.zero(st));
    if (a->n_rows) {
        AssembleArgs aa = assemble_args(a->lazy_dict, a->lazy_rows, a, d_flag.p);
        { StageTimer t(ctx, &ctx->tm.assemble); launch_assemble_lazy(a, aa, st, 1); }
        SKX_HIP(hipMemcpyAsync(a->vcount.p, a->present.p, a->n_rows * 4, hipMemcpyDeviceToDevice, st));
    }
    SKX_TRY(check_missing(ctx, d_flag.p));
    a->stats_ready = true;
    return SKX_OK;
}

int skx::array_lazy_rows(skx_array *a, uint8_t *out, uint64_t pitch, uint32_t j_base, uint32_t n_blocks, uint64_t col_base, const uint8_t *keep, const uint64_t *kpos,
                         int mask_ambig, bool full_pieces)
{
    skx_ctx *ctx = a->ctx; hipStream_t st = ctx->stream;
    if (a->pieces) {
        const skx_pieces *pc = a->pieces; const skx_keyset *rows = a->lazy_rows;
        PiecesRowsArgs pa{};
        pa.pieces = pc->data.p; pa.plen = pc->plen.p; pa.perm = pc->perm.p; pa.nrank = pc->nrank.p; pa.cap = pc->cap; pa.n_samples = (int)a->names.size();
        pa.ncnt = rows->ncnt.p; pa.roff = rows->roff.p;
        pa.out = out; pa.pitch = pitch; pa.j_base = j_base; pa.col_base = col_base;
        pa.keep = keep; pa.kpos = kpos; pa.mask_ambig = mask_ambig; pa.full_pieces = full_pieces ? 1 : 0;
        const uint32_t nb = n_blocks ? n_blocks : 1u << pc->logQ;
        if (keep) { KernelTimer kt(ctx, &ctx->tm.pieces_rows); launch_pieces_rows(pa, nb, st); }
        else { StageTimer t(ctx, &ctx->tm.assemble); launch_pieces_rows(pa, nb, st); }
        SKX_HIP(hipGetLastError());
        return SKX_OK;
    }
    DevBuf<int> d_flag; SKX_TRY(d_flag.alloc(1)); SKX_TRY(d_flag.zero(st));
    AssembleArgs aa = assemble_args(a->lazy_dict, a->lazy_rows, a, d_flag.p);
    aa.matrix = out; aa.pitch = pitch; aa.j_base = j_base; aa.col_base = col_base;
    aa.keep = keep; aa.kpos = kpos; aa.mask_ambig = mask_ambig;
    { StageTimer t(ctx, &ctx->tm.assemble); launch_assemble_lazy(a, aa, st, keep ? 2 : 0, n_blocks); }
    return check_missing(ctx, d_flag.p);
}
int skx::array_materialize(skx_array *a)
{
    if (!a->lazy()) return SKX_OK;
    skx_ctx *ctx = a->ctx; hipStream_t st = ctx->stream;
    SKX_HIP(hipSetDevice(ctx->device));
    if (a->pieces) SKX_TRY(array_lazy_stats(a));
    const uint64_t U = a->n_rows;
    a->pitch = pitch_for(U);
    SKX_TRY(a->matrix.alloc((uint64_t)a->names.size() * a->pitch));
    if (U) {
        SKX_TRY(array_lazy_rows(a, a->matrix.p, a->pitch));
        if (!a->stats_ready) SKX_HIP(hipMemcpyAsync(a->vcount.p, a->present.p, U * 4, hipMemcpyDeviceToDevice, st));
    }
    SKX_HIP(hipStreamSynchronize(st));
    SKX_HIP(hipGetLastError());
    a->stats_ready = true;
    a->drop_lazy();
    return SKX_OK;
}
int skx::array_lazy_window(skx_array *a, uint64_t r0, uint64_t nr, DevBuf<uint8_t> &buf, const uint8_t **win, uint64_t *wpitch)
{
    skx_keyset *rows = a->lazy_rows;
    if (rows->h_roff.empty()) {
        rows->h_roff.resize((1ull << rows->logN) + 1);
        SKX_HIP(hipMemcpy(rows->h_roff.data(), rows->roff.p, rows->h_roff.size() * 8, hipMemcpyDeviceToHost));
    }
    const auto &ro = rows->h_roff;
    const uint64_t j0 = (uint64_t)(std::upper_bound(ro.begin(), ro.end(), r0) - ro.begin()) - 1;
    const uint64_t j1 = (uint64_t)(std::lower_bound(ro.begin(), ro.end(), r0 + nr) - ro.begin());
    const uint64_t c0 = ro[j0] & ~15ull, span = ro[j1] - c0;
    const uint64_t wp = pitch_for(span);
    const size_t S = a->names.size();
    if (buf.n < S * wp) SKX_TRY(buf.alloc(S * wp));
    SKX_TRY(array_lazy_rows(a, buf.p, wp, (uint32_t)j0, (uint32_t)(j1 - j0), c0));
    *win = buf.p + (r0 - c0); *wpitch = wp;
    return SKX_OK;
}

extern "C" int skx_merge(skx_ctx *ctx, skx_dictset *d, const char *const *names, skx_array **out)
{
    return skx_guarded([&]() -> int {
    if (!ctx || !d || !out) { set_error("bad arguments"); return SKX_EINVAL; }
    { const int ra = merge_append(ctx, d, names, out); if (ra != SKF_NOT_TAKEN) return ra; }
    SKX_TRY(dictset_sort(d));
    skx_keyset *ks = nullptr;
    SKX_TRY(keyset_union_dict(ctx, d, &ks, true));
    int r = skx_array_assemble(ctx, d, ks, names, out);
    skx_keyset_free(ks);
    return r;
    });
}

int skx::merge_batch(skx_ctx *ctx, skx_dictset *d, const char *const *names, skx_array **out)
{
    const auto t0 = std::chrono::steady_clock::now();
    int r = merge_append(ctx, d, names, out);
    if (r == SKF_NOT_TAKEN && !knob("eager_array")) {
        skx_keyset *ks = nullptr;
        r = skx_keyset_union(ctx, d, &ks);
        if (r == SKX_OK) r = array_make_lazy(ctx, d, ks, names, out); else skx_dictset_free(d);
        d = nullptr;
    } else if (r == SKF_NOT_TAKEN)
        r = skx_merge(ctx, d, names, out);
    const auto t1 = std::chrono::steady_clock::now();
    skx_dictset_free(d);
    phase_add("build.merge", std::chrono::duration<double>(t1 - t0).count());
    phase_add("build.release_dictionaries", std::chrono::duration<double>(std::chrono::steady_clock::now() - t1).count());
    return r;
}
```

Measured before the change: 31090.

## Add two-tier append table spilling late rows to a global hash tier

Adds a two-tier mode to the append kernel. Each block's LDS hash table closes once it holds enough rows, and rows that arrive later go to a per-block global-memory hash table (tier 2), with their presence bits buffered in a per-wave LDS list and flushed to the pieces. At finalisation the two tiers are sorted separately and merged by binary search. A host-side planner turns this on when early samples dominate the row count, which lets the split use one fewer logQ level (fewer, larger row blocks) and so re-read regions less often. The cost is global atomics, extra fences and resyncs, and more complex finalisation.

```diff
diff --git a/ska.rust_amd/csrc/skx_append.hip b/ska.rust_amd/csrc/skx_append.hip
--- a/ska.rust_amd/csrc/skx_append.hip
+++ b/ska.rust_amd/csrc/skx_append.hip
@@ -80,26 +80,31 @@
 
 typedef volatile uint32_t __attribute__((address_space(3))) *lds_vol_t;
 __device__ static inline lds_vol_t lds_vol(void *p) { return (lds_vol_t)(__attribute__((address_space(3))) void *)p; }
-constexpr int CTL_NROWS = 0, CTL_FAIL = 1, CTL_TMP = 8, CTL_WORDS = 32;
-
-static inline size_t append_lds_bytes(uint32_t nslots, uint32_t cap, bool count_only)
+constexpr int CTL_NROWS = 0, CTL_FAIL = 1, CTL_CLOSED = 2, CTL_NLDS = 3, CTL_CLOSE_IT = 4, CTL_TMP = 8, CTL_WORDS = 32;
+constexpr uint32_t T2_TOTAL = APPEND_T2_SLOTS + APPEND_T2_PAD, T2_SHIFT = 32u - 14u;
+static_assert(APPEND_T2_SLOTS == 1u << 14, "T2_SHIFT");
+
+size_t append_lds_bytes(uint32_t nslots, uint32_t rb_ranks, bool count_only, bool two_tier)
 {
     size_t b = (size_t)(nslots + AP_PAD) * 8 + (size_t)(nslots + AP_PAD) + (size_t)AP_WAVES * (AP_Q + AP_SQ) * 8 + CTL_WORDS * 4;
-    if (!count_only) b += (size_t)AP_WAVES * (cap / 8) * 4;
+    if (!count_only) b += (size_t)AP_WAVES * (rb_ranks / 8) * 4;
+    if (two_tier) b += (size_t)AP_WAVES * APPEND_TT_LIST * 4;
     return b;
 }
 
-template <bool COUNT_ONLY, bool HI>
+template <bool COUNT_ONLY, bool HI, bool TT = false>
 __global__ __launch_bounds__(AP_THREADS) void append_kernel(AppendArgs a)
 {
+    static_assert(!(COUNT_ONLY && TT), "the count-only form has one tier");
     extern __shared__ __attribute__((aligned(16))) unsigned char s_raw[];
     const uint32_t total_slots = a.nslots + AP_PAD;
-    const uint32_t cap = a.cap, rbw = cap / 8;
+    const uint32_t cap = a.cap, rbcap = TT ? a.rb_ranks : cap, rbw = rbcap / 8;
     unsigned char *s_fp = s_raw;
     unsigned long long *s_tab = reinterpret_cast<unsigned long long *>(s_raw + total_slots);
-    unsigned long long *s_q = s_tab + total_slots;
-    uint32_t *s_ctl = reinterpret_cast<uint32_t *>(s_q + (size_t)AP_WAVES * (AP_Q + AP_SQ));
-    uint32_t *s_rb = s_ctl + CTL_WORDS;
+    uint32_t *s_ctl = reinterpret_cast<uint32_t *>(s_tab + total_slots + (TT ? 0 : (size_t)AP_WAVES * (AP_Q + AP_SQ)));
+    unsigned long long *s_q = TT ? reinterpret_cast<unsigned long long *>(s_ctl + CTL_WORDS) : s_tab + total_slots;
+    uint32_t *s_rb = TT ? reinterpret_cast<uint32_t *>(s_q + (size_t)AP_WAVES * (AP_Q + AP_SQ)) : s_ctl + CTL_WORDS;
+    uint32_t *s_list = s_rb + (size_t)AP_WAVES * rbw;
     const int tid = threadIdx.x, lane = tid & 63;
     const int wv = __builtin_amdgcn_readfirstlane(tid >> 6);
     const int S = a.n_samples;
@@ -116,6 +121,8 @@
     uint8_t *piece0 = nullptr;
     unsigned long long *q = s_q + (size_t)wv * (AP_Q + AP_SQ), *sq = q + AP_Q;
     uint32_t *rb = s_rb + (size_t)wv * rbw;
+    unsigned long long *const t2 = TT ? a.t2 + (size_t)blockIdx.x * T2_TOTAL : nullptr;
+    uint32_t *const lst = s_list + (size_t)wv * APPEND_TT_LIST;
     for (uint32_t rnd = 0; rnd < a.rounds; rnd++) {
     if (xmap) {
         const uint32_t xcd = blockIdx.x & 7u, ls = blockIdx.x >> 3, gpr = (G >> 3) >> shA;
@@ -128,12 +135,14 @@
     for (uint32_t i = tid; i < total_slots; i += AP_THREADS) s_tab[i] = 0ull;
     for (uint32_t i = tid; i < total_slots / 4u; i += AP_THREADS) reinterpret_cast<uint32_t *>(s_fp)[i] = 0u;
     if (!COUNT_ONLY) for (uint32_t i = tid; i < AP_WAVES * rbw; i += AP_THREADS) s_rb[i] = 0u;
-    if (tid < CTL_WORDS) s_ctl[tid] = 0u;
+    if (tid < CTL_WORDS) s_ctl[tid] = TT && tid == CTL_CLOSED && a.lds_close == 0u ? 1u : 0u;
+    if (TT) for (uint32_t i = tid; i < T2_TOTAL; i += AP_THREADS) __hip_atomic_store(&t2[i], 0ull, __ATOMIC_RELAXED, __HIP_MEMORY_SCOPE_AGENT);
     if (tid == 0 && (uint32_t)(uintptr_t)(__attribute__((address_space(3))) unsigned char *)s_fp != 0u) atomicOr(a.overflow, 4);
     if (xmap && A > 1u && a.bar && tid == 0) {
         atomicAdd(&a.bar[region], 1);
         for (int it = 0; it < (1 << 18) && __hip_atomic_load(&a.bar[region], __ATOMIC_RELAXED, __HIP_MEMORY_SCOPE_AGENT) < (int)A; it++) __builtin_amdgcn_s_sleep(8);
     }
+    if (TT) __threadfence();
     __syncthreads();
 
     typedef const uint64_t __attribute__((address_space(4))) *cq_t;
@@ -143,6 +152,8 @@
     const uint64_t rstride = 1ull << a.logB;
     const uint32_t qbase = (uint32_t)(uintptr_t)(__attribute__((address_space(3))) unsigned long long *)q, qfull = qbase + 128u * 8u;
     uint32_t qw = qbase, nsq = 0;
+    int s_cur = wv;
+    uint32_t nl = 0, filled = 0;
     AP_PROF_START;
     __builtin_amdgcn_s_setprio(AP_PRIO_STREAM);
 
@@ -161,11 +172,26 @@
         const uint32_t rank = rank1 - 1u;
         atomicOr(&rb[rank >> 3], m4 << ((rank & 7u) * 4u));
     };
+    auto list_out = [&](uint32_t n, uint8_t *dst) {
+        const uint32_t g0 = filled > rbcap / 32u ? filled : rbcap / 32u, g1 = (n + 31u) / 32u;
+        for (uint32_t g = g0 + (uint32_t)lane; g < g1; g += 64u) *reinterpret_cast<uint4 *>(dst + (size_t)g * 16u) = make_uint4(0u, 0u, 0u, 0u);
+        if (g1 > g0) filled = g1;
+        if (nl) {
+            asm volatile("s_waitcnt vmcnt(0)" ::: "memory");
+            if ((uint32_t)lane < nl) {
+                const uint32_t e = lst[lane], rank = e >> 4;
+                atomicOr(reinterpret_cast<uint32_t *>(dst) + (rank >> 3), (e & 15u) << ((rank & 7u) * 4u));
+            }
+            nl = 0;
+        }
+    };
     auto slow_batch = [&]() {
         __builtin_amdgcn_s_setprio(AP_PRIO_INSERT);
         const uint32_t take = nsq < 64u ? nsq : 64u;
         nsq -= take;
         if (lane == 0) { AP_COUNT(8, 1); AP_COUNT(9, take); }
+        const bool closed = TT && lds_vol(&s_ctl[CTL_CLOSED])[0] != 0u;
+        uint32_t far_cell = 0;
         if ((uint32_t)lane < take) {
             const unsigned long long w = sq[nsq + lane];
             const uint32_t wlo = (uint32_t)w, whi = (uint32_t)(w >> 32);
@@ -180,14 +206,16 @@
                 uint32_t at = 0;
                 if (!(m0 | m1 | m2 | m3)) {
                     at = e0 == 0ull ? 0u : e1 == 0ull ? 1u : e2 == 0ull ? 2u : e3 == 0ull ? 3u : 4u;
-                    if (at < 4u) won = atomicCAS(&s_tab[t + at], 0ull, keyE | AP_RANK_MASK) == 0ull;
+                    if (TT && closed) { if (at < 4u) break; }
+                    else if (at < 4u) won = atomicCAS(&s_tab[t + at], 0ull, keyE | AP_RANK_MASK) == 0ull;
                 }
                 if (won) {
                     const uint32_t mine = atomicAdd(&s_ctl[CTL_NROWS], 1u) + 1u;
-                    if (mine > (COUNT_ONLY ? AP_RANK_MASK - 1u : cap)) s_ctl[CTL_FAIL] = 1u;
-                    lds_vol(&s_tab[t + at])[0] = kl | (mine < AP_RANK_MASK ? mine : AP_RANK_MASK - 1u);
+                    if (mine > (COUNT_ONLY ? AP_RANK_MASK - 1u : rbcap)) s_ctl[CTL_FAIL] = 1u;
+                    if (TT) lds_vol(&s_tab[t + at])[0] = kl | (mine <= rbcap ? mine : rbcap);
+                    else lds_vol(&s_tab[t + at])[0] = kl | (mine < AP_RANK_MASK ? mine : AP_RANK_MASK - 1u);
                     s_fp[t + at] = (unsigned char)key_fp(kh, kl);
-                    rank1 = mine;
+                    rank1 = TT && mine > rbcap ? rbcap : mine;
                 }
                 __builtin_amdgcn_wave_barrier();
                 if (m0 | m1 | m2 | m3) {
@@ -201,9 +229,46 @@
                 if (won) break;
                 if (at == 4u) t += 4u;
             }
+            if (TT && closed && rank1 == 0) {
+                for (uint32_t t = kh >> T2_SHIFT; t < T2_TOTAL; t++) {
+                    const unsigned long long e = atomicCAS(&t2[t], 0ull, keyE | AP_RANK_MASK);
+                    const bool won = e == 0ull;
+                    if (won) {
+                        const uint32_t mine = atomicAdd(&s_ctl[CTL_NROWS], 1u) + 1u;
+                        if (mine > cap) s_ctl[CTL_FAIL] = 1u;
+                        __hip_atomic_store(&t2[t], keyE | (mine <= cap ? mine : cap), __ATOMIC_RELAXED, __HIP_MEMORY_SCOPE_AGENT);
+                        rank1 = mine;
+                    }
+                    __builtin_amdgcn_wave_barrier();
+                    if (!won && (e ^ keyE) - 1ull < AP_RANK_MASK) {
+                        uint32_t r = (uint32_t)e & AP_RANK_MASK;
+                        for (int it = 0; it < (1 << 16) && r == AP_RANK_MASK; it++) r = (uint32_t)__hip_atomic_load(&t2[t], __ATOMIC_RELAXED, __HIP_MEMORY_SCOPE_AGENT) & AP_RANK_MASK;
+                        if (r == AP_RANK_MASK) r = 0;
+                        rank1 = r;
+                        break;
+                    }
+                    if (won) break;
+                }
+            }
             if (rank1 > cap && !COUNT_ONLY) rank1 = 0;
             if (rank1 == 0) s_ctl[CTL_FAIL] = 1u;
-            else if (!COUNT_ONLY) record(rank1, wlo & 15u);
+            else if (!COUNT_ONLY) {
+                if (!TT || rank1 <= rbcap) record(rank1, wlo & 15u);
+                else far_cell = (((rank1 - 1u) << 4) | (wlo & 15u)) + 1u;
+            }
+        }
+        if (TT) {
+            for (unsigned long long pend = __ballot(far_cell != 0u); pend; pend = __ballot(far_cell != 0u)) {
+                if (nl == APPEND_TT_LIST) {
+                    uint32_t n = *lds_vol(&s_ctl[CTL_NROWS]);
+                    n = __builtin_amdgcn_readfirstlane(n);
+                    list_out(n < cap ? n : cap, piece0 + (uint64_t)s_cur * (cap / 2));
+                    if (lane == 0 && a.tt_stat) atomicAdd(&a.tt_stat[4], 1ull);
+                }
+                const uint32_t room = APPEND_TT_LIST - nl, idx = ap_mbcnt(pend), cnt = (uint32_t)__popcll(pend);
+                if (far_cell && idx < room) { lst[nl + idx] = far_cell - 1u; far_cell = 0u; }
+                nl += cnt < room ? cnt : room;
+            }
         }
         __builtin_amdgcn_s_setprio(AP_PRIO_STREAM);
     };
@@ -385,26 +450,34 @@
                     n = __builtin_amdgcn_readfirstlane(n);
                     if (n > cap) n = cap;
                     uint8_t *dst = piece0 + (uint64_t)s * (cap / 2);
-                    for (uint32_t v = lane; v * 32u < n; v += 64u) {
+                    const uint32_t nb = TT && n > rbcap ? rbcap : n;
+                    for (uint32_t v = lane; v * 32u < nb; v += 64u) {
                         uint4 *src = reinterpret_cast<uint4 *>(rb) + v;
                         const uint4 x = *src;
                         *reinterpret_cast<uint4 *>(dst + v * 16u) = x;
                         *src = make_uint4(0u, 0u, 0u, 0u);
                     }
+                    if (TT) { list_out(n, dst); filled = 0; }
                     if (lane == 0) a.plen[j * (uint64_t)S + s] = (uint16_t)n;
                 }
                 AP_PROF(4);
                 if (!more) break;
                 s += AP_WAVES; c = 0; off_c = off_n; cnt_c = cnt_n;
+                s_cur = s;
                 if (AP_RESYNC > 0) {
                     const int it = (s - wv) / AP_WAVES;
-                    if (xmap && A > 1u && a.bar && it % (AP_RESYNC > 0 ? AP_RESYNC : 1) == 0 && it <= (S - AP_WAVES) / AP_WAVES) {
+                    const int rs = TT ? (int)a.resync : (AP_RESYNC > 0 ? AP_RESYNC : 1);
+                    const bool readers_meet = xmap && A > 1u && a.bar;
+                    if ((TT || readers_meet) && it % rs == 0 && it <= (S - AP_WAVES) / AP_WAVES) {
                         __syncthreads();
                         if (tid == 0) {
-                            int *ctr = a.bar + (1 << a.logB) + region;
-                            const int want = (int)A * (it / (AP_RESYNC > 0 ? AP_RESYNC : 1));
-                            atomicAdd(ctr, 1);
-                            for (int spin = 0; spin < (1 << 16) && __hip_atomic_load(ctr, __ATOMIC_RELAXED, __HIP_MEMORY_SCOPE_AGENT) < want; spin++) __builtin_amdgcn_s_sleep(4);
+                            if (TT && !s_ctl[CTL_CLOSED] && s_ctl[CTL_NROWS] >= a.lds_close) { s_ctl[CTL_CLOSED] = 1u; s_ctl[CTL_NLDS] = s_ctl[CTL_NROWS]; s_ctl[CTL_CLOSE_IT] = (uint32_t)it; }
+                            if (readers_meet) {
+                                int *ctr = a.bar + (1 << a.logB) + region;
+                                const int want = (int)A * (it / rs);
+                                atomicAdd(ctr, 1);
+                                for (int spin = 0; spin < (1 << 16) && __hip_atomic_load(ctr, __ATOMIC_RELAXED, __HIP_MEMORY_SCOPE_AGENT) < want; spin++) __builtin_amdgcn_s_sleep(4);
+                            }
                         }
                         __syncthreads();
                     }
@@ -423,6 +496,87 @@
         for (uint32_t i = tid; i < total_slots; i += AP_THREADS) c += s_tab[i] != 0ull;
         uint32_t tot; (void)ap_block_excl(c, s_tmp, &tot);
         if (tid == 0) { atomicAdd(&a.probe[0], (unsigned long long)tot); atomicMax(&a.probe[1], (unsigned long long)tot); }
+        continue;
+    }
+    if (TT) {
+        unsigned long long *s_l1 = s_q, *s_l2 = s_tab;
+        uint16_t *s_perm = reinterpret_cast<uint16_t *>(s_q + rbcap);
+        for (uint32_t i = tid; i < cap; i += AP_THREADS) s_perm[i] = 0xFFFFu;
+        const uint32_t per = (total_slots + AP_THREADS - 1) / AP_THREADS;
+        const uint32_t lo = tid * per < total_slots ? tid * per : total_slots, hi = lo + per < total_slots ? lo + per : total_slots;
+        uint32_t c = 0;
+        for (uint32_t i = lo; i < hi; i++) c += s_tab[i] != 0ull;
+        uint32_t n1;
+        uint32_t pos = ap_block_excl(c, s_tmp, &n1);
+        for (uint32_t i = lo; i < hi; i++) {
+            const unsigned long long e = s_tab[i];
+            if (!e) continue;
+            uint32_t gl = 0, lr = 0;
+            for (int64_t t = (int64_t)i - 1; t >= 0; t--) { const unsigned long long o = s_tab[t]; if (!o) break; gl += o > e; }
+            for (uint32_t t = i + 1; t < total_slots; t++) { const unsigned long long o = s_tab[t]; if (!o) break; lr += o < e; }
+            const uint32_t idx = pos - gl + lr;
+            pos++;
+            if (idx < rbcap) s_l1[idx] = e;
+        }
+        constexpr uint32_t per2 = (T2_TOTAL + AP_THREADS - 1) / AP_THREADS;
+        const uint32_t lo2 = tid * per2 < T2_TOTAL ? tid * per2 : T2_TOTAL, hi2 = lo2 + per2 < T2_TOTAL ? lo2 + per2 : T2_TOTAL;
+        auto t2_at = [&](uint32_t i) { return __hip_atomic_load(&t2[i], __ATOMIC_RELAXED, __HIP_MEMORY_SCOPE_AGENT); };
+        unsigned long long v2[per2];
+#pragma unroll
+        for (uint32_t i = 0; i < per2; i++) v2[i] = lo2 + i < hi2 ? t2_at(lo2 + i) : 0ull;
+        c = 0;
+#pragma unroll
+        for (uint32_t i = 0; i < per2; i++) c += v2[i] != 0ull;
+        uint32_t n2;
+        uint32_t pos2 = ap_block_excl(c, s_tmp, &n2);
+        const bool fits = n1 <= rbcap && n2 <= total_slots && n1 + n2 <= a.stride;
+        if (!fits) { if (tid == 0) atomicOr(a.overflow, 1); __syncthreads(); continue; }
+#pragma unroll
+        for (uint32_t i = 0; i < per2; i++) {
+            const unsigned long long e = v2[i];
+            if (e) {
+                uint32_t gl = 0, lr = 0;
+                bool open = true;
+#pragma unroll
+                for (uint32_t t = i; t-- > 0;) { open = open && v2[t] != 0ull; gl += open && v2[t] > e; }
+                if (open) for (int64_t t = (int64_t)lo2 - 1; t >= 0; t--) { const unsigned long long o = t2_at((uint32_t)t); if (!o) break; gl += o > e; }
+                open = true;
+#pragma unroll
+                for (uint32_t t = i + 1; t < per2; t++) { open = open && v2[t] != 0ull; lr += open && v2[t] < e; }
+                if (open && lo2 + per2 == hi2) for (uint32_t t = hi2; t < T2_TOTAL; t++) { const unsigned long long o = t2_at(t); if (!o) break; lr += o < e; }
+                s_l2[pos2 - gl + lr] = e;
+                pos2++;
+            }
+        }
+        __syncthreads();
+        uint64_t *slab = a.stage + j * (uint64_t)a.stride;
+        auto below = [&](const unsigned long long *v, uint32_t n, unsigned long long e) -> uint32_t {
+            uint32_t l = 0, h = n;
+            while (l < h) { const uint32_t m = (l + h) >> 1; if (v[m] < e) l = m + 1; else h = m; }
+            return l;
+        };
+        auto place = [&](unsigned long long e, uint32_t idx) {
+            const uint32_t rank = ((uint32_t)e & AP_RANK_MASK) - 1u;
+            if (idx >= a.stride || rank >= cap) return;
+            uint64_t hl;
+            if (HI) hl = ((uint64_t)(uint32_t)(e >> 32) << lowb) | (uint64_t)((uint32_t)e >> AP_RANK_BITS);
+            else hl = rem == 0 ? 0ull : (uint64_t)((uint32_t)(e >> 32) >> (32 - rem));
+            slab[idx] = ((((uint64_t)j << rem) | hl) << 4) | 1ull;
+            s_perm[rank] = (uint16_t)idx;
+        };
+        for (uint32_t i = tid; i < n1; i += AP_THREADS) { const unsigned long long e = s_l1[i]; place(e, i + below(s_l2, n2, e)); }
+        for (uint32_t i = tid; i < n2; i += AP_THREADS) { const unsigned long long e = s_l2[i]; place(e, i + below(s_l1, n1, e)); }
+        __syncthreads();
+        uint16_t *pj = a.perm + j * (uint64_t)cap;
+        for (uint32_t i = tid; i < cap; i += AP_THREADS) pj[i] = s_perm[i];
+        if (tid == 0) {
+            a.ncnt[j] = n1 + n2; a.nrank[j] = nr < cap ? nr : cap;
+            if (a.tt_stat) {
+                if (s_ctl[CTL_CLOSED]) { atomicAdd(&a.tt_stat[0], 1ull); atomicAdd(&a.tt_stat[1], (unsigned long long)s_ctl[CTL_NLDS]); atomicMax(&a.tt_stat[3], (unsigned long long)s_ctl[CTL_CLOSE_IT]); }
+                atomicAdd(&a.tt_stat[2], (unsigned long long)n2);
+            }
+        }
+        __syncthreads();
         continue;
     }
     uint16_t *s_perm = reinterpret_cast<uint16_t *>(s_q);
@@ -462,8 +616,21 @@
 template <bool COUNT_ONLY>
 static void launch_append_t(const AppendArgs &a, unsigned blocks, hipStream_t st)
 {
-    const size_t lds = append_lds_bytes(a.nslots, a.cap, COUNT_ONLY);
     const bool hi = a.bits - a.logQ >= 32;
+    if constexpr (!COUNT_ONLY) {
+        if (a.two_tier) {
+            const size_t lds = append_lds_bytes(a.nslots, a.rb_ranks, false, true);
+            if (hi) {
+                (void)hipFuncSetAttribute((const void *)append_kernel<false, true, true>, hipFuncAttributeMaxDynamicSharedMemorySize, (int)lds);
+                hipLaunchKernelGGL((append_kernel<false, true, true>), dim3(blocks), dim3(AP_THREADS), lds, st, a);
+            } else {
+                (void)hipFuncSetAttribute((const void *)append_kernel<false, false, true>, hipFuncAttributeMaxDynamicSharedMemorySize, (int)lds);
+                hipLaunchKernelGGL((append_kernel<false, false, true>), dim3(blocks), dim3(AP_THREADS), lds, st, a);
+            }
+            return;
+        }
+    }
+    const size_t lds = append_lds_bytes(a.nslots, a.cap, COUNT_ONLY, false);
     if (hi) {
         (void)hipFuncSetAttribute((const void *)append_kernel<COUNT_ONLY, true>, hipFuncAttributeMaxDynamicSharedMemorySize, (int)lds);
         hipLaunchKernelGGL((append_kernel<COUNT_ONLY, true>), dim3(blocks), dim3(AP_THREADS), lds, st, a);
@@ -472,12 +639,15 @@
         hipLaunchKernelGGL((append_kernel<COUNT_ONLY, false>), dim3(blocks), dim3(AP_THREADS), lds, st, a);
     }
 }
-bool append_ok(int bits, int logB, int logQ, uint32_t region_cap, uint32_t nslots, uint32_t cap)
+bool append_ok(int bits, int logB, int logQ, uint32_t region_cap, uint32_t nslots, uint32_t cap, uint32_t tt_rb_ranks)
 {
     const int rem = bits - logQ;
     (void)region_cap;
-    return logQ >= logB && rem >= 0 && rem <= 50 && cap % 128u == 0 && cap >= 128u && cap <= APPEND_MAX_CAP && nslots >= cap && (nslots & (nslots - 1u)) == 0u &&
-           append_lds_bytes(nslots, cap, false) <= 160u * 1024u - 256u;
+    if (!(logQ >= logB && rem >= 0 && rem <= 50 && cap % 128u == 0 && cap >= 128u && (nslots & (nslots - 1u)) == 0u)) return false;
+    if (tt_rb_ranks)
+        return cap <= APPEND_MAX_RANKS && tt_rb_ranks % 128u == 0 && tt_rb_ranks >= 128u && tt_rb_ranks <= cap && tt_rb_ranks <= APPEND_TT_LDS_RANKS && nslots >= tt_rb_ranks &&
+               append_lds_bytes(nslots, tt_rb_ranks, false, true) <= 160u * 1024u - 256u;
+    return cap <= APPEND_MAX_CAP && nslots >= cap && append_lds_bytes(nslots, cap, false, false) <= 160u * 1024u - 256u;
 }
 void launch_append(const AppendArgs &a, uint32_t region_cap, hipStream_t st) { (void)region_cap; launch_append_t<false>(a, (1u << a.logQ) / a.rounds, st); }
 void launch_append_probe(const AppendArgs &a, uint32_t region_cap, unsigned blocks, hipStream_t st) { (void)region_cap; launch_append_t<true>(a, blocks, st); }
@@ -559,14 +729,18 @@
         if (rc < lim) lim = rc;
     }
     const uint32_t nseen = (lim + 31u) / 32u * 32u < nr ? (lim + 31u) / 32u * 32u : nr;
-    const uint32_t ncol = (lim + 31u) / 32u, ncg = ncol < 64u ? ncol : 64u;
+    const uint32_t ncol_all = (lim + 31u) / 32u;
+    const uint32_t nturn = gridDim.y == 1 && ncol_all > 256u ? (ncol_all + 255u) / 256u : 1u;
+    const uint16_t *pj = perm + j * (uint64_t)cap;
+    for (uint32_t turn = 0; turn < nturn; turn++) {
+    const uint32_t ncol = ncol_all - turn * 256u < 256u || !staged ? ncol_all - turn * 256u : 256u, ncg = ncol < 64u ? ncol : 64u;
     uint32_t G = 4, P = 1;
     if (staged && ncol) {
         G = (ncol + 63u) / 64u;
-        for (P = 4u / G; P > 1u && (P / 2u) * G * 36u * 4u * ncg > PS_STAGE * 6u; P >>= 1) { }
+        for (P = nturn > 1u ? 1u : 4u / G; P > 1u && (P / 2u) * G * 36u * 4u * ncg > PS_STAGE * 6u; P >>= 1) { }
     }
     const uint32_t grp = (uint32_t)wv % G, slice = (uint32_t)wv / G;
-    const uint32_t d = blockIdx.y * 256u + grp * 64u + (uint32_t)lane;
+    const uint32_t d = (blockIdx.y + turn) * 256u + grp * 64u + (uint32_t)lane;
     const uint4 *col = reinterpret_cast<const uint4 *>(pieces + j * (uint64_t)S * (cap / 2)) + d;
     const uint32_t step = cap / 32;
     bool mine = slice < P && d * 32u < lim;
@@ -648,11 +822,10 @@
         }
         if (slice) mine = false;
     }
-    if (staged) {
+    if (staged && turn == 0) {
         for (uint32_t p = threadIdx.x; p < nrows; p += 256) { s_pr[p] = 0; s_un[p] = 0; s_mk[p] = 0; }
         __syncthreads();
     }
-    const uint16_t *pj = perm + j * (uint64_t)cap;
     if (mine) {
 #pragma unroll
         for (int w = 0; w < W; w++) {
@@ -681,9 +854,10 @@
             }
         }
     }
+    }
     if (!staged) __threadfence();
     __syncthreads();
-    const uint32_t rk0 = blockIdx.y * 256u * 8u * W, rk1 = rk0 + 256u * 8u * W < nseen ? rk0 + 256u * 8u * W : nseen;
+    const uint32_t rk0 = blockIdx.y * 256u * 8u * W, rk1 = rk0 + 256u * 8u * W < nseen && gridDim.y > 1 ? rk0 + 256u * 8u * W : nseen;
     for (uint32_t rb = rk0 + (uint32_t)wv * 64u; rb < rk1; rb += 256u) {
         const uint32_t rr = rb + (uint32_t)lane;
         uint32_t pp = 0xFFFFu; bool hit = false;
@@ -724,7 +898,7 @@
 StatsLaunch stats_launch(uint32_t cap)
 {
     static const int direct = knob("stats_direct") ? 1 : 0;
-    return {(cap / 32 + 255u) / 256u, direct, (cap + 63u) / 64u * 64u};
+    return {cap <= APPEND_MAX_RANKS ? 1u : (cap / 32 + 255u) / 256u, direct, (cap + 63u) / 64u * 64u};
 }
 }
 void launch_pieces_stats(const uint8_t *pieces, const uint16_t *plen, const uint16_t *perm, const uint32_t *nrank, const uint32_t *ncnt, const uint64_t *roff, uint32_t cap,
@@ -733,6 +907,7 @@
     if (n_blocks <= 0) return;
     const StatsLaunch l = stats_launch(cap);
     if (!l.bounded()) min_count = 0;
+    if ((size_t)l.stage * 6 > 48u * 1024u) (void)hipFuncSetAttribute((const void *)pieces_stats_kernel, hipFuncAttributeMaxDynamicSharedMemorySize, (int)((size_t)l.stage * 6));
     hipLaunchKernelGGL(pieces_stats_kernel, dim3((unsigned)n_blocks, l.gy), dim3(256), (size_t)l.stage * 6, st, pieces, plen, perm, nrank, ncnt, roff, cap, n_samples, present, unambig, mask, vcount,
                        l.direct, l.stage, min_count, tally);
 }
@@ -892,7 +1067,8 @@
     if (!n_blocks || a.n_samples <= 0) return;
     PiecesRowsArgs b = a;
     int spw = a.n_samples;
-    while (spw > PR_WAVES * 4 && (uint64_t)n_blocks * ((a.n_samples + spw - 1) / spw) < 8192) spw = (spw + 1) / 2;
+    const uint64_t want = a.cap > APPEND_MAX_SLOTS ? 4096 : 8192;
+    while (spw > PR_WAVES * 4 && (uint64_t)n_blocks * ((a.n_samples + spw - 1) / spw) < want) spw = (spw + 1) / 2;
     b.samples_per_wg = spw;
     const unsigned gy = (unsigned)((a.n_samples + spw - 1) / spw);
     const size_t lds = (((size_t)a.cap + 16) * 2 + 15) / 16 * 16 + (size_t)PR_WAVES * (a.cap / 8 + 4) * 4;
diff --git a/ska.rust_amd/csrc/skx_device.h b/ska.rust_amd/csrc/skx_device.h
--- a/ska.rust_amd/csrc/skx_device.h
+++ b/ska.rust_amd/csrc/skx_device.h
@@ -140,6 +140,8 @@
                             uint16_t *side, uint16_t *perm, hipStream_t st);
 
 constexpr uint32_t APPEND_MAX_CAP = 6016, APPEND_MAX_SLOTS = 8192;
+constexpr uint32_t APPEND_MAX_RANKS = 12032, APPEND_TT_LDS_RANKS = 5760, APPEND_TT_LIST = 32, APPEND_T2_SLOTS = 16384, APPEND_T2_PAD = 64;
+constexpr int APPEND_TT_STATS = 8;
 struct AppendArgs {
     const uint64_t *words; const uint64_t *off; const uint32_t *raw;
     int n_samples, logB, bits, logQ;
@@ -150,8 +152,15 @@
     int *overflow;
     uint32_t rounds = 1;
     int *bar = nullptr;
-};
-bool append_ok(int bits, int logB, int logQ, uint32_t region_cap, uint32_t nslots, uint32_t cap);
+    int two_tier = 0;
+    uint32_t rb_ranks = 0;
+    uint32_t lds_close = 0;
+    uint32_t resync = 0;
+    unsigned long long *t2 = nullptr;
+    unsigned long long *tt_stat = nullptr;
+};
+size_t append_lds_bytes(uint32_t nslots, uint32_t rb_ranks, bool count_only, bool two_tier);
+bool append_ok(int bits, int logB, int logQ, uint32_t region_cap, uint32_t nslots, uint32_t cap, uint32_t tt_rb_ranks = 0);
 void launch_append(const AppendArgs &a, uint32_t region_cap, hipStream_t st);
 void launch_append_probe(const AppendArgs &a, uint32_t region_cap, unsigned blocks, hipStream_t st);
 constexpr uint32_t APPEND_WIDE_MAX_CAP = 3072, APPEND_WIDE_MAX_SLOTS = 4096;
diff --git a/ska.rust_amd/csrc/skx_merge.cpp b/ska.rust_amd/csrc/skx_merge.cpp
--- a/ska.rust_amd/csrc/skx_merge.cpp
+++ b/ska.rust_amd/csrc/skx_merge.cpp
@@ -295,12 +295,14 @@
     }
 }
 
-struct AppendSplit { uint32_t cap, nslots; uint64_t amp; bool allowed; uint32_t rounds; uint64_t grid; };
-static AppendSplit append_split(double u_est, double est_relvar, int logQ, int logB, uint32_t region_cap, bool wide, int cus, uint64_t raw_sum)
+struct AppendSplit { uint32_t cap, nslots; uint64_t amp; bool allowed; uint32_t rounds; uint64_t grid; uint32_t rb_ranks; };
+static AppendSplit append_split(double u_est, double est_relvar, int logQ, int logB, uint32_t region_cap, bool wide, int cus, uint64_t raw_sum, bool two_tier = false)
 {
     AppendSplit s{};
     const uint64_t nsub = 1ull << logQ;
-    s.cap = ranks_for(u_est / (double)nsub, est_relvar, append_max_cap(wide)); s.nslots = slots_for(s.cap, append_max_slots(wide));
+    s.cap = ranks_for(u_est / (double)nsub, est_relvar, two_tier ? APPEND_MAX_RANKS : append_max_cap(wide));
+    s.rb_ranks = two_tier ? std::min(s.cap, APPEND_TT_LDS_RANKS) : s.cap;
+    s.nslots = slots_for(s.rb_ranks, append_max_slots(wide));
     s.amp = 1ull << (logQ - logB);
     const uint64_t amp_max = region_cap > lds_sort_max(wide) ? 32 : 8;
     s.allowed = !(s.amp > amp_max && (double)raw_sum * (double)s.amp > 4e8);
@@ -309,6 +311,34 @@
     const bool persistent = g <= (uint64_t)std::max(cus, 1) && nsub % g == 0 && g % (8 * s.amp) == 0 && logB >= 3;
     s.grid = persistent ? g : 0; s.rounds = persistent ? (uint32_t)(nsub / g) : 1;
     return s;
+}
+
+constexpr double TT_HOT = 0.5, TT_NEW = 0.02, TT_FULL = 0.8;
+struct TwoTierPlan { bool on = false; uint32_t lds_close = 0, resync = 16; };
+static TwoTierPlan two_tier_plan(double u_est, double est_relvar, uint64_t raw_max, int S, int logQ_fine, int min_logQ)
+{
+    TwoTierPlan p;
+    p.resync = (uint32_t)std::min(16, std::max(1, S / 64));
+    if (logQ_fine - 1 < min_logQ || S < 2) return p;
+    if ((int)p.resync > (S - 16) / 16) return p;
+    const double nsub = (double)(1ull << (logQ_fine - 1));
+    const double first = (double)raw_max / nsub, per = std::max(0.0, u_est - (double)raw_max) / nsub / (double)(S - 1), between = 16.0 * p.resync * per;
+    if (ranks_need(u_est / nsub, est_relvar) > (double)APPEND_MAX_RANKS) return p;
+    if (first > TT_HOT * (double)APPEND_TT_LDS_RANKS) return p;
+    if (per > TT_NEW * first) return p;
+    if (ranks_need(first + between, est_relvar) > (double)APPEND_TT_LDS_RANKS) return p;
+    if (u_est / (2.0 * nsub) < TT_FULL * (double)APPEND_MAX_CAP) return p;
+    p.lds_close = (uint32_t)std::max(1.0, (double)APPEND_TT_LDS_RANKS - ranks_need(between, 0.0));
+    p.on = true;
+    return p;
+}
+
+extern "C" int skx_debug_two_tier_plan(double u_est, double est_relvar, uint64_t raw_max, int n_samples, int logQ_fine, int min_logQ, uint32_t *out)
+{
+    if (!out) { set_error("bad arguments"); return SKX_EINVAL; }
+    const TwoTierPlan p = two_tier_plan(u_est, est_relvar, raw_max, n_samples, logQ_fine, min_logQ);
+    out[0] = p.on ? 1u : 0u; out[1] = p.lds_close; out[2] = p.resync;
+    return SKX_OK;
 }
 
 static int append_pass(skx_ctx *ctx, skx_dictset *d, std::unique_ptr<skx_keyset> &ks_out, std::unique_ptr<skx_pieces> &pc_out)
@@ -331,14 +361,21 @@
     SKX_TRY(estimate_rows(ctx, d, aa, min_logQ, raw_max, e));
     int logQ = min_logQ;
     while (logQ < bits && ranks_need(e.u_est / (double)(1ull << logQ), e.est_relvar) > (double)append_max_cap(wide)) logQ++;
+    const long tt_knob = wide || knob("append_two_tier", 1) == 0 ? 0 : knob("append_lds_ranks");
+    TwoTierPlan tt;
+    if (!wide && knob("append_two_tier", 1) != 0 && tt_knob <= 0) tt = two_tier_plan(e.u_est, e.est_relvar, raw_max, S, logQ, min_logQ);
+    if (tt.on) logQ--;
+    if (tt_knob > 0) { tt.lds_close = tt_knob <= 1 ? 0u : (uint32_t)tt_knob; tt.resync = 1; }
     if (knob("append_coarse") > 0) logQ = std::max<long>(min_logQ, logQ - knob("append_coarse"));
     int cus = 0; (void)hipDeviceGetAttribute(&cus, hipDeviceAttributeMultiprocessorCount, ctx->device);
     for (int attempt = 0;; attempt++, logQ++) {
-        if (logQ > bits || attempt > 3) return append_not_taken(ctx, "row blocks kept overflowing (a sample that is one repeat, or far more rows than the probe saw)");
+        const bool two = tt_knob > 0 || (tt.on && attempt == 0);
+        if (logQ > bits || attempt > (tt.on ? 4 : 3)) return append_not_taken(ctx, "row blocks kept overflowing (a sample that is one repeat, or far more rows than the probe saw)");
         const uint64_t nsub = 1ull << logQ;
-        const AppendSplit sp = append_split(e.u_est, e.est_relvar, logQ, logB, d->region_cap, wide, cus, raw_sum);
+        const AppendSplit sp = append_split(e.u_est, e.est_relvar, logQ, logB, d->region_cap, wide, cus, raw_sum, two);
         if (!sp.allowed) return append_not_taken(ctx, "too many row blocks per region: every region would be read too often");
-        if (!append_fits(wide, bits, logB, logQ, d->region_cap, sp.nslots, sp.cap)) return append_not_taken(ctx, "no row-block split that fits the LDS");
+        if (!(two ? append_ok(bits, logB, logQ, d->region_cap, sp.nslots, sp.cap, sp.rb_ranks) : append_fits(wide, bits, logB, logQ, d->region_cap, sp.nslots, sp.cap)))
+            return append_not_taken(ctx, "no row-block split that fits the LDS");
         std::unique_ptr<skx_keyset> ks(new skx_keyset());
         ks->ctx = ctx; ks->k = d->k; ks->rc = d->rc; ks->logN = logQ; ks->hp = d->hp; ks->wh = d->wh; ks->wide = wide; ks->stride = sp.cap;
         std::unique_ptr<skx_pieces> pc(new skx_pieces());
@@ -352,12 +389,26 @@
         aa.logQ = logQ; aa.nslots = sp.nslots; aa.cap = sp.cap; aa.rounds = sp.rounds; aa.bar = d_bar.p;
         aa.pieces = pc->data.p; aa.plen = pc->plen.p; aa.perm = pc->perm.p; aa.nrank = pc->nrank.p;
         aa.stage = ks->stage.p; aa.stride = sp.cap; aa.ncnt = ks->ncnt.p;
+        DevBuf<unsigned long long> d_t2, d_tts;
+        aa.two_tier = two ? 1 : 0; aa.rb_ranks = sp.rb_ranks; aa.lds_close = tt.lds_close; aa.resync = tt.resync; aa.t2 = nullptr; aa.tt_stat = nullptr;
+        if (two) {
+            const uint64_t wgs = nsub / sp.rounds;
+            if (d_t2.alloc(wgs * (uint64_t)(APPEND_T2_SLOTS + APPEND_T2_PAD)) != SKX_OK) return append_not_taken(ctx, "no room for the second tier");
+            SKX_TRY(d_tts.alloc(APPEND_TT_STATS)); SKX_TRY(d_tts.zero(st));
+            aa.t2 = d_t2.p; aa.tt_stat = d_tts.p;
+        }
         { KernelTimer kt(ctx, &ctx->tm.append); if (wide) launch_append_wide(aa, st); else launch_append(aa, d->region_cap, st); }
         int ov = 0;
+        unsigned long long tts[APPEND_TT_STATS] = {};
         SKX_HIP(hipMemcpyAsync(&ov, d_flag.p, 4, hipMemcpyDeviceToHost, st));
+        if (two && getenv("SKX_DEBUG")) SKX_HIP(hipMemcpyAsync(tts, d_tts.p, sizeof tts, hipMemcpyDeviceToHost, st));
         SKX_HIP(hipStreamSynchronize(st));
         SKX_HIP(hipGetLastError());
-        if (getenv("SKX_DEBUG")) fprintf(stderr, "[skx] append%s: logQ=%d (x%llu per region) cap=%u slots=%u rows~%.0f -> %s [sized by %s]\n", wide ? " (128-bit keys)" : "", logQ, (unsigned long long)sp.amp, sp.cap, sp.nslots, e.u_est, ov ? "overflow" : "ok", e.sized);
+        if (getenv("SKX_DEBUG")) {
+            fprintf(stderr, "[skx] append%s: logQ=%d (x%llu per region) cap=%u slots=%u rows~%.0f -> %s [sized by %s]\n", wide ? " (128-bit keys)" : "", logQ, (unsigned long long)sp.amp, sp.cap, sp.nslots, e.u_est, ov ? "overflow" : "ok", e.sized);
+            if (two) fprintf(stderr, "[skx] append two tiers: %s split, lds_ranks=%u close_at=%u meet_every=%u closed_blocks=%llu of %llu lds_rows=%llu last_close_meeting=%llu tier2_rows=%llu list_flushes=%llu\n",
+                             tt.on ? "coarser" : "same", sp.rb_ranks, tt.lds_close, tt.resync, tts[0], (unsigned long long)nsub, tts[1], tts[3], tts[2], tts[4]);
+        }
         if (ov & 4) return append_not_taken(ctx, "the table's bytes are not at LDS address 0");
         if (ov) continue;
         SKX_TRY(keyset_finish(ks.get()));
```

Result: faster. 32330, median of 6 (+4.0%).
